# Totoro97/f2-nerf

Measured on AMD Instinct MI355X. Metric: training ray-samples/s (ngp_fox), higher is better.
Workload: dtype f16; 1 GPU; ngp_fox wanjinyou.yaml, 8192 rays/batch/GPU, 2^19 x16 table, the first 2188 iterations of training from the fresh-initialised table (fineness 8.7), synthetic random-pose rays, full train step (fwd+bwd+Adam+octree update); rays_per_batch=8192, parallelism=ray-dp1

## Files before the change

### f2-nerf_amd/capi.py

```python
import ctypes
import os

import torch

from . import build

_lib = None
ABI_VERSION = 13


class F2nError(RuntimeError):
    pass


def lib():
    global _lib
    if _lib is None:
        if not os.path.exists(build.LIB):
            raise F2nError("native library %s is missing: run `python -c 'import __graft_entry__ as g; g.build()'` "
                           "(there is no CPU fallback)" % build.LIB)
        _lib = ctypes.CDLL(build.LIB)
        _lib.f2n_build_info.restype = ctypes.c_char_p
        if _lib.f2n_abi_version() != ABI_VERSION:
            raise F2nError("%s reports ABI version %d, this binding is written for %d: rebuild (__graft_entry__.build())"
                           % (build.LIB, _lib.f2n_abi_version(), ABI_VERSION))
    return _lib


def _stream():
    return ctypes.c_void_p(torch.cuda.current_stream().cuda_stream)


_DT = {"f32": torch.float32, "i32": torch.int32, "i64": torch.int64, "u8": torch.uint8, "h16": torch.float16}


def _p(t, kind=None, allow_none=False):
    if t is None:
        if allow_none:
            return ctypes.c_void_p(0)
        raise F2nError("required tensor is None")
    if not t.is_cuda:
# ... 141 lines not shown
                                    _p(noise, "f32"), _p(oct_se, "i32"), _p(oct_idx, "i32"), _p(oct_nf, "f32"), _p(tree_nodes, "u8"),
                                    _p(transes, "u8"), _p(counts, "i32"), _p(s_pts, "f32", True), _p(s_dt, "f32"), _p(s_t, "f32"),
                                    _p(s_anchors, "i32"), _p(first_oct_dis, "f32"), _p(oct_trans, "i32", True)), "f2n_ray_march_strided")


def pack_samples(n_rays, pts_se, rays_o, rays_d, transes, s_pts, s_dt, s_t, s_anchors, pts, dirs, dt, t, anchors):
    _ck(lib().f2n_pack_samples(_stream(), _i(n_rays), _p(pts_se, "i32"), _p(rays_o, "f32", True), _p(rays_d, "f32"),
                               _p(transes, "u8", True), _p(s_pts, "f32", True), _p(s_dt, "f32"),
                               _p(s_t, "f32"), _p(s_anchors, "i32"), _p(pts, "f32"), _p(dirs, "f32"), _p(dt, "f32"), _p(t, "f32"),
                               _p(anchors, "i32")), "f2n_pack_samples")


def pack_samples_repair(n_rays, pts_se, rays_o, rays_d, transes, s_pts, s_dt, s_t, s_anchors, pts, dirs, dt, t, anchors, death_epoch,
                        spec_epoch):
    _ck(lib().f2n_pack_samples_repair(_stream(), _i(n_rays), _p(pts_se, "i32"), _p(rays_o, "f32", True), _p(rays_d, "f32"),
                                      _p(transes, "u8", True), _p(s_pts, "f32", True), _p(s_dt, "f32"), _p(s_t, "f32"),
                                      _p(s_anchors, "i32"), _p(pts, "f32"), _p(dirs, "f32"), _p(dt, "f32"), _p(t, "f32"),
                                      _p(anchors, "i32"), _p(death_epoch, "i32"), _i(spec_epoch)), "f2n_pack_samples_repair")


def edge_samples(n, edge_pool, transes, edge_idx, edge_coords, out_pts, out_idx):
    _ck(lib().f2n_edge_samples(_stream(), _i(n), _p(edge_pool, "u8"), _p(transes, "u8"), _p(edge_idx, "i32"),
                               _p(edge_coords, "f32"), _p(out_pts, "f32"), _p(out_idx, "i32")), "f2n_edge_samples")


def early_stop_votes(n_rays, pts_se, f0, f0_stride, dt, weights, alphas, mask, kept, anchors, anchor_stride, w_adder, a_adder, mark,
                     visit_cnt):
    _ck(lib().f2n_early_stop_votes(_stream(), _i(n_rays), _p(pts_se, "i32"), _p(f0, "f32"), _i(f0_stride), _p(dt, "f32"),
                                   _p(weights, "f32"), _p(alphas, "f32"), _p(mask, "i32"), _p(kept, "i32"), _i(w_adder.numel()),
                                   _p(anchors, "i32"), _i(anchor_stride), _p(w_adder, "i32"), _p(a_adder, "i32"), _p(mark, "i32"),
                                   _p(visit_cnt, "i32")), "f2n_early_stop_votes")


def oct_mark_visit(n_rays, pts_se, anchors, anchor_stride, weights, alphas, w_adder, a_adder, mark, visit_cnt):
    _ck(lib().f2n_oct_mark_visit(_stream(), _i(n_rays), _i(w_adder.numel()), _p(pts_se, "i32"), _p(anchors, "i32"), _i(anchor_stride),
                                 _p(weights, "f32"), _p(alphas, "f32"), _p(w_adder, "i32"), _p(a_adder, "i32"),
                                 _p(mark, "i32"), _p(visit_cnt, "i32")), "f2n_oct_mark_visit")


def oct_update_stats(n_nodes, w_adder, a_adder, mark, w_stats, a_stats, tree_nodes, child_blocks=None, reset_votes=False):
    _ck(lib().f2n_oct_update_stats(_stream(), _i(n_nodes), _p(w_adder, "i32"), _p(a_adder, "i32"), _p(mark, "i32"),
                                   _p(w_stats, "i32"), _p(a_stats, "i32"), _p(tree_nodes, "u8"),
                                   _p(child_blocks, "u8", True), _i(1 if reset_votes else 0)), "f2n_oct_update_stats")


def oct_update_stats_ex(n_nodes, w_adder, a_adder, mark, w_stats, a_stats, tree_nodes, child_blocks, reset_votes, died_at, epoch,
                        death_epoch):
    _ck(lib().f2n_oct_update_stats_ex(_stream(), _i(n_nodes), _p(w_adder, "i32"), _p(a_adder, "i32"), _p(mark, "i32"),
                                      _p(w_stats, "i32"), _p(a_stats, "i32"), _p(tree_nodes, "u8"), _p(child_blocks, "u8", True),
                                      _i(int(reset_votes)), _p(died_at, "i32", True), _i(epoch), _p(death_epoch, "i32", True),
                                      ctypes.c_void_p(0)), "f2n_oct_update_stats_ex")


def oct_intersect_repair(n_rays, max_hits, search_order, rays_o, rays_d, near, far, tree_nodes, oct_se, oct_idx, oct_nf, total,
                         oct_trans, child_blocks, died_at, spec_epoch, death_epoch, repair_flags, n_repaired=None):
    _ck(lib().f2n_oct_intersect_repair(_stream(), _i(n_rays), _i(max_hits), _p(search_order, "u8"), _p(rays_o, "f32"),
                                       _p(rays_d, "f32"), _f(near), _f(far), _p(tree_nodes, "u8"), _p(oct_se, "i32"),
                                       _p(oct_idx, "i32"), _p(oct_nf, "f32"), _p(total, "i32"), _p(oct_trans, "i32", True),
                                       _p(child_blocks, "u8", True), _p(died_at, "i32"), _i(spec_epoch), _p(death_epoch, "i32"),
                                       _p(repair_flags, "i32"), _p(n_repaired, "i32", True)), "f2n_oct_intersect_repair")


def ray_march_repair(n_rays, sample_l, scale_by_dis, rays_o, rays_d, noise, oct_se, oct_idx, oct_nf, tree_nodes, transes, counts,
                     s_pts, s_dt, s_t, s_anchors, first_oct_dis, oct_trans, repair_flags, death_epoch, spec_epoch):
    _ck(lib().f2n_ray_march_repair(_stream(), _i(n_rays), _f(sample_l), _i(int(scale_by_dis)), _p(rays_o, "f32"), _p(rays_d, "f32"),
                                   _p(noise, "f32"), _p(oct_se, "i32"), _p(oct_idx, "i32"), _p(oct_nf, "f32"), _p(tree_nodes, "u8"),
# ... 226 lines not shown


def draw_ray_batch(n_rays, u01, image_set, height, width, poses, intri, dist_params, images, cam_bounds, cam_indices, ij, rays_o,
                   rays_d, gt_colors, bounds):
    _ck(lib().f2n_draw_ray_batch(_stream(), _i(n_rays), _p(u01, "f32"), _p(image_set, "i32"), _i(int(image_set.numel())), _i(height),
                                 _i(width), _p(poses, "f32"), _p(intri, "f32"), _p(dist_params, "f32"), _p(images, "f32", True),
                                 _p(cam_bounds, "f32"), _p(cam_indices, "i32"), _p(ij, "i32"), _p(rays_o, "f32"), _p(rays_d, "f32"),
                                 _p(gt_colors, "f32", True), _p(bounds, "f32")), "f2n_draw_ray_batch")


def gather_pixels(n, height, width, images, cam_bounds, cam_idx, ij, gt_colors, bounds):
    _ck(lib().f2n_gather_pixels(_stream(), _i(n), _i(height), _i(width), _p(images, "f32", True), _p(cam_bounds, "f32", True),
                                _p(cam_idx, "i32"), _p(ij, "i32"), _p(gt_colors, "f32", True), _p(bounds, "f32", True)),
        "f2n_gather_pixels")


def early_stop(n_rays, pts_se, f0, f0_stride, dt, weights, alphas, mask, kept):
    _ck(lib().f2n_early_stop(_stream(), _i(n_rays), _p(pts_se, "i32"), _p(f0, "f32"), _i(f0_stride), _p(dt, "f32"),
                             _p(weights, "f32"), _p(alphas, "f32"), _p(mask, "i32"), _p(kept, "i32")), "f2n_early_stop")


def compact_samples(n_rays, old_se, new_se, mask, pts, dirs, dt, t, anchors, o_pts, o_dirs, o_dt, o_t, o_anchors):
    _ck(lib().f2n_compact_samples(_stream(), _i(n_rays), _p(old_se, "i32"), _p(new_se, "i32"), _p(mask, "i32"),
                                  _p(pts, "f32"), _p(dirs, "f32"), _p(dt, "f32"), _p(t, "f32"), _p(anchors, "i32"),
                                  _p(o_pts, "f32"), _p(o_dirs, "f32"), _p(o_dt, "f32"), _p(o_t, "f32"),
                                  _p(o_anchors, "i32")), "f2n_compact_samples")


def compact_samples_src(n_rays, old_se, new_se, mask, pts, dirs, dt, t, anchors, o_pts, o_dirs, o_dt, o_t, o_anchors, o_src,
                        o_vol=None, ray_val=None, o_ray_val=None):
    _ck(lib().f2n_compact_samples_src(_stream(), _i(n_rays), _p(old_se, "i32"), _p(new_se, "i32"), _p(mask, "i32"),
                                      _p(pts, "f32"), _p(dirs, "f32"), _p(dt, "f32"), _p(t, "f32"), _p(anchors, "i32"),
                                      _p(o_pts, "f32"), _p(o_dirs, "f32"), _p(o_dt, "f32"), _p(o_t, "f32"),
                                      _p(o_anchors, "i32"), _p(o_src, "i32"), _p(o_vol, "i32", True), _p(ray_val, "i32", True),
                                      _p(o_ray_val, "i32", True)), "f2n_compact_samples_src")


def oct_visible_cams(n_boxes, n_cams, boxes, c2w, bounds, fx, fy, cx, cy, res_h, res_w, pix_i, pix_j, visible):
    _ck(lib().f2n_oct_visible_cams(_stream(), _i(n_boxes), _i(n_cams), _p(boxes, "f32"), _p(c2w, "f32"), _p(bounds, "f32"), _f(fx),
                                   _f(fy), _f(cx), _f(cy), _i(res_h), _i(res_w), _p(pix_i, "f32"), _p(pix_j, "f32"),
                                   _p(visible, "u8")), "f2n_oct_visible_cams")


def march_noise(n, u, fineness, out):
    _ck(lib().f2n_march_noise(_stream(), _i(n), _p(u, "f32"), _f(fineness), _p(out, "f32")), "f2n_march_noise")


def composite_fwd(n_rays, pts_se, feat, dt, t, rgb, bg, colors, disparity, depth, weights, f0_stride=16, out_vars=None):
    _ck(lib().f2n_composite_fwd(_stream(), _i(n_rays), _p(pts_se, "i32"), _p(feat, "f32"), _i(f0_stride), _p(dt, "f32"),
                                _p(t, "f32"), _p(rgb, "f32"), _p(bg, "f32"), _p(colors, "f32"), _p(disparity, "f32"),
                                _p(depth, "f32"), _p(weights, "f32"), _p(out_vars, "f32", True)), "f2n_composite_fwd")


def composite_bwd(n_rays, pts_se, feat, dt, t, rgb, bg, dcolors, ddisp, ddepth, dweights, gs_progress, drgb, dfeat, f0_stride=16,
                  df0_stride=16, var_weights=None, dvars=None):
    _ck(lib().f2n_composite_bwd(_stream(), _i(n_rays), _p(pts_se, "i32"), _p(feat, "f32"), _i(f0_stride), _p(dt, "f32"),
                                _p(t, "f32"), _p(rgb, "f32"), _p(bg, "f32"), _p(dcolors, "f32", True), _p(ddisp, "f32", True),
                                _p(ddepth, "f32", True), _p(dweights, "f32", True), _f(gs_progress), _p(drgb, "f32"),
                                _p(dfeat, "f32"), _i(df0_stride), _p(var_weights, "f32", True), _p(dvars, "f32", True)),
        "f2n_composite_bwd")


def weight_var_fwd(n_rays, weights, pts_se, out):
    _ck(lib().f2n_weight_var_fwd(_stream(), _i(n_rays), _p(weights, "f32"), _p(pts_se, "i32"), _p(out, "f32")),
        "f2n_weight_var_fwd")


# ... 156 lines not shown


def reduce_deferred():
    _ck(lib().f2n_reduce_deferred(_stream()), "f2n_reduce_deferred")


def deferred_reset():
    _ck(lib().f2n_deferred_reset(), "f2n_deferred_reset")


def adam_step_h16grad(n, param, grad_h, grad_scale, exp_avg, exp_avg_sq, step, lr, beta1, beta2, eps, wd, param_h,
                      zero_grad, skip_flag=None):
    _ck(lib().f2n_adam_step_h16grad(_stream(), _i(n), _p(param, "f32"), _p(grad_h, "h16"), _f(grad_scale),
                                    _p(exp_avg, "f32"), _p(exp_avg_sq, "f32"), _i(step), _f(lr), _d(beta1), _d(beta2),
                                    _f(eps), _f(wd), _p(param_h, "h16"), _i(int(zero_grad)),
                                    _p(skip_flag, "i32", True)), "f2n_adam_step_h16grad")


def train_loss(n_rays, pred, gt, disparity, sampled_var, n_edge, feat_dim, edge_feats, var_w, disp_w, tv_w, out_losses,
               dcolors, ddisparity, dvar, dedge_feats):
    _ck(lib().f2n_train_loss(_stream(), _i(n_rays), _p(pred, "f32"), _p(gt, "f32"), _p(disparity, "f32", True),
                             _p(sampled_var, "f32", True), _i(n_edge), _i(feat_dim), _p(edge_feats, "f32", True), _f(var_w),
                             _f(disp_w), _f(tv_w), _p(out_losses, "f32"), _p(dcolors, "f32", True), _p(ddisparity, "f32", True),
                             _p(dvar, "f32", True), _p(dedge_feats, "f32", True)), "f2n_train_loss")


def composite_train(n_rays, se, f0, f0_stride, dt, t, rgb, bg, gt, var_w, disp_w, tv_w, gs_progress, n_edge, feat_dim, edge_feats,
                    dedge_feats, colors, weights, drgb, df0, df0_stride, out_losses, defer_reduce=False):
    _ck(lib().f2n_composite_train(_stream(), _i(n_rays), _p(se, "i32"), _p(f0, "f32"), _i(f0_stride), _p(dt, "f32"), _p(t, "f32"),
                                  _p(rgb, "f32"), _p(bg, "f32"), _p(gt, "f32"), _f(var_w), _f(disp_w), _f(tv_w), _f(gs_progress),
                                  _i(n_edge), _i(feat_dim), _p(edge_feats, "f32", True), _p(dedge_feats, "f32", True),
                                  _p(colors, "f32"), _p(weights, "f32"), _p(drgb, "f32"), _p(df0, "f32"), _i(df0_stride),
                                  _p(out_losses, "f32"), _i(1 if defer_reduce else 0)), "f2n_composite_train")


def nonfinite_flags(n_a, a, n_b, b, flags, mirror=None):
    _ck(lib().f2n_nonfinite_flags_ex(_stream(), _i(n_a), _p(a, "f32", True), _i(n_b), _p(b, "f32", True), _p(flags, "i32"),
                                     _mapped(mirror)), "f2n_nonfinite_flags_ex")


def _lo3(lo):
    return (_f * 3)(*(float(v) for v in lo))


def oct_locate_warp(n, pts_world, tree_nodes, transes, out_pts, out_anchors):
    _ck(lib().f2n_oct_locate_warp(_stream(), _i(n), _p(pts_world, "f32"), _p(tree_nodes, "u8"), _p(transes, "u8"), _p(out_pts, "f32"),
                                  _p(out_anchors, "i32")), "f2n_oct_locate_warp")


def oct_locate_warp_grid(lo, step, nx, ny, nz, first_z, n_z, tree_nodes, transes, out_pts, out_anchors):
    _ck(lib().f2n_oct_locate_warp_grid(_stream(), _lo3(lo), _f(step), _i(nx), _i(ny), _i(nz), _i(first_z), _i(n_z), _p(tree_nodes, "u8"),
                                       _p(transes, "u8"), _p(out_pts, "f32"), _p(out_anchors, "i32")), "f2n_oct_locate_warp_grid")


def located_compact(n, anchors, pts_warped, counts, start_end, total, out_pts, out_vol, out_src=None):
    _ck(lib().f2n_located_compact(_stream(), _i(n), _p(anchors, "i32"), _p(pts_warped, "f32"), _p(counts, "i32"), _p(start_end, "i32"),
                                  _p(total, "i32"), _p(out_pts, "f32"), _p(out_vol, "i32"), _p(out_src, "i32", True)),
        "f2n_located_compact")


def density_scatter(n, anchors, start_end, f0, density):
    _ck(lib().f2n_density_scatter(_stream(), _i(n), _p(anchors, "i32"), _p(start_end, "i32"), _p(f0, "f32"), _p(density, "f32")),
        "f2n_density_scatter")


def field_density_grad(n, n_volumes, table_h, prim_pool, local_idx, local_size, bias_pool, level_scale, pts_warped, volume_idx, vol_stride,
# ... 552 lines not shown
```

### f2-nerf_amd/csrc/host/PersSampler.cpp

```cpp
#include "PersSampler.h"

#include <hip/hip_runtime_api.h>

#include <algorithm>
#include <cstring>
#include <functional>

namespace f2n {

namespace {

Tensor BuildSearchOrder() {
  std::vector<int> search_order;
  for (int st = 0; st < 8; st++) {
    auto cmp = [st](int a, int b) {
      int bt = ((a ^ b) & -(a ^ b));
      return ((a & bt) ^ (st & bt)) != 0;
    };
    for (int i = 0; i < 8; i++) search_order.push_back(i);
    std::sort(search_order.begin() + st * 8, search_order.begin() + (st + 1) * 8, cmp);
  }
  return torch::from_blob(search_order.data(), {64}, CpuI32()).to(torch::kUInt8).to(torch::kCUDA).contiguous();
}

// ... 289 lines not shown
  F2N_CALL(f2n_edge_samples(CurStream(), n_pts, VoidP(pers_octree_->edge_pool_gpu_), VoidP(pers_octree_->pers_trans_gpu_),
                            I32P(edge_idx), F32P(edge_coord), F32P(out_pts), I32P(out_idx)));
  return {out_pts, out_idx};
}

Tensor& PersSampler::VoteBuffer() {
  auto& oct = *pers_octree_;
  const int n_nodes = oct.n_nodes_;
  Tensor& occ = oct.occ_;
  if (!occ.defined() || occ.size(1) != n_nodes || oct.tree_visit_cnt_.data_ptr() != (void*) (occ.data_ptr<int32_t>() + 3 * (int64_t) n_nodes)) {
    occ = torch::empty({4, n_nodes}, DevI32());
    occ.slice(0, 0, 2).fill_(-1);
    occ.select(0, 2).zero_();
    occ.select(0, 3).copy_(oct.tree_visit_cnt_);
    oct.tree_visit_cnt_ = occ.select(0, 3);
  }
  return occ;
}

void PersSampler::UpdateOctNodes(const SampleResultFlex& sample_result, const Tensor& sampled_weight,
                                 const Tensor& sampled_alpha) {
  const int n_nodes = pers_octree_->n_nodes_;
  const int n_rays = sample_result.pts_idx_bounds.size(0);
  CheckDev(sampled_weight, torch::kFloat32, "sampled_weight");
  CheckDev(sampled_alpha, torch::kFloat32, "sampled_alpha");
  Tensor& occ = VoteBuffer();
  F2N_TIMED_CALL("oct_mark_visit", f2n_oct_mark_visit(CurStream(), n_rays, n_nodes, I32P(sample_result.pts_idx_bounds), I32P(sample_result.anchors), 3,
                              F32P(sampled_weight), F32P(sampled_alpha), I32P(occ), I32P(occ) + n_nodes,
                              I32P(occ) + 2 * (int64_t) n_nodes, I32P(occ) + 3 * (int64_t) n_nodes));
  FinishOctUpdate();
}

void PersSampler::EarlyStopAndVote(const SampleResultFlex& sample_result, const float* f0, Tensor& weights, Tensor& alphas, Tensor& mask,
                                   Tensor& kept) {
  const int n_nodes = pers_octree_->n_nodes_;
  const int n_rays = sample_result.pts_idx_bounds.size(0);
  Tensor& occ = VoteBuffer();
  F2N_TIMED_CALL("early_stop", f2n_early_stop_votes(CurStream(), n_rays, I32P(sample_result.pts_idx_bounds), f0, 1, F32P(sample_result.dt),
                              F32P(weights), F32P(alphas), I32P(mask), I32P(kept), n_nodes, I32P(sample_result.anchors), 3, I32P(occ),
                              I32P(occ) + n_nodes, I32P(occ) + 2 * (int64_t) n_nodes, I32P(occ) + 3 * (int64_t) n_nodes));
}

void PersSampler::FinishOctUpdate(const ScanArgs* scan) {
  auto& oct = *pers_octree_;
  const int n_nodes = oct.n_nodes_;
  Tensor& occ = oct.occ_;
  void* st = CurStream();
  if (occupancy_sync_hook_) occupancy_sync_hook_(occ);
  Tensor adders = occ.slice(0, 0, 2), visit_mark = occ.select(0, 2);
  oct.epoch_++;
  if (scan != nullptr) {
    F2N_TIMED_CALL("oct_update_stats", f2n_oct_update_stats_scan(st, n_nodes, I32P(adders), I32P(adders) + n_nodes, I32P(visit_mark),
                                  I32P(oct.tree_weight_stats_), I32P(oct.tree_alpha_stats_), VoidP(oct.tree_nodes_gpu_),
                                  VoidP(oct.child_blocks_gpu_), 1, I32P(oct.died_at_), oct.epoch_, I32P(oct.death_epoch_),
                                  oct.death_epoch_host_dev_, scan->n, scan->counts, scan->start_end, scan->total, scan->mirror, scan->also,
                                  scan->n_also));
  } else {
    F2N_TIMED_CALL("oct_update_stats", f2n_oct_update_stats_ex(st, n_nodes, I32P(adders), I32P(adders) + n_nodes, I32P(visit_mark),
                                  I32P(oct.tree_weight_stats_), I32P(oct.tree_alpha_stats_), VoidP(oct.tree_nodes_gpu_),
                                  VoidP(oct.child_blocks_gpu_), 1, I32P(oct.died_at_), oct.epoch_, I32P(oct.death_epoch_),
                                  oct.death_epoch_host_dev_));
  }

  while (!sub_div_milestones_.empty() && sub_div_milestones_.back() <= global_data_pool_->iter_step_) {
    oct.ProcOctree(true, true, sub_div_milestones_.back() <= 0);
    oct.MarkInvisibleNodes();
    oct.ProcOctree(true, false, false);
    sub_div_milestones_.pop_back();
  }
  if (global_data_pool_->iter_step_ % compact_freq_ == 0) {
    oct.ProcOctree(true, false, false);
  }
}
// ... 113 lines not shown
```

### f2-nerf_amd/csrc/host/PersSampler.h

```cpp
#pragma once
#include <functional>

#include "KeyedDraws.h"
#include "MappedHost.h"
#include "PtsSampler.h"

namespace f2n {

#define INIT_NODE_STAT 1000
#define N_PROS 12

struct alignas(32) TransInfo {
  float w2xz[N_PROS][2][4];
  float weight[3][N_PROS];
  float center[3];
  float dis_summary;
};
struct alignas(32) TreeNode {
  float center[3];
  float side_len;
  int parent;
  int childs[8];
  bool is_leaf_node;
  int trans_idx;
// ... 52 lines not shown
  at::cuda::CUDAEvent counts_ready;
  bool speculative = false, completed = true;
  bool packed_once = false;
  int spec_epoch = 0;
  int64_t generation = 0;
  Tensor repair_flags;
  Tensor leaf_state, reached;
  bool tail = false;
};

class PersSampler : public PtsSampler {
 public:
  explicit PersSampler(GlobalDataPool* global_data_pool);
  SampleResultFlex GetSamples(const Tensor& rays_o, const Tensor& rays_d, const Tensor& bounds) override;
  void BeginSamples(const Tensor& rays_o, const Tensor& rays_d, float fineness, PendingSamples& p, bool speculative = false,
                    int64_t seq = -1);
  int64_t keyed_seq_ = -1;
  bool CompleteSpeculative(PendingSamples& p);
  void IssueScanAndPack(PendingSamples& p);
  void IssueScan(PendingSamples& p);
  bool tail_repair_ = true;
  int march_blocks_ = 512;
  int march_block_waves_ = 4;
  bool persistent_march_ = false;
  int LdsWalkMaxInterior() const { return f2n_oct_lds_max_interior(); }
  bool MaintenanceDue(int ahead = 0) const;
  bool MaintenanceDueAt(int iter) const;
  SampleResultFlex FinishSamples(PendingSamples& p);
  std::tuple<Tensor, Tensor> GetEdgeSamples(int n_pts) override;
  std::tuple<Tensor, Tensor> LocatePoints(const Tensor& world);
  void UpdateOctNodes(const SampleResultFlex& sample_result, const Tensor& sampled_weights,
                      const Tensor& sampled_alpha) override;
  void EarlyStopAndVote(const SampleResultFlex& sample_result, const float* f0, Tensor& weights, Tensor& alphas, Tensor& mask,
                        Tensor& kept);
  struct ScanArgs {
    int n = 0;
    const int32_t* counts = nullptr;
    int32_t *start_end = nullptr, *total = nullptr, *mirror = nullptr;
    const int32_t* also = nullptr;
    int n_also = 0;
  };
  void FinishOctUpdate(const ScanArgs* scan = nullptr);
  Tensor& VoteBuffer();
  MappedWords totals_words_;
  int next_totals_slot_ = 0;
  std::vector<Tensor> States() override;
  int LoadStates(const std::vector<Tensor>& states, int idx) override;

  void InstallOctree(const Tensor& tree_nodes_bytes, const Tensor& pers_trans_bytes, const Tensor& edge_pool_bytes);
  void SetEdgePool(const Tensor& edge_pool_bytes);
  void SetTrainCameras(const Tensor& w2c, const Tensor& intri, const Tensor& bounds);

  std::unique_ptr<PersOctree> pers_octree_;
  std::vector<int> sub_div_milestones_;
  int compact_freq_;
  int max_oct_intersect_per_ray_;
  float global_near_;
  float sample_l_;
  bool scale_by_dis_;
  std::function<void(Tensor)> occupancy_sync_hook_;
  Tensor forced_noise_, forced_edge_idx_, forced_edge_coords_;
  KeyedUniforms noise_draws_{0x9E3779B97F4A7C15ull};
  int extra_sample_rows_ = 0;
};

}
```

### f2-nerf_amd/csrc/host/Renderer.cpp

```cpp
#include "Renderer.h"

#include <hip/hip_runtime_api.h>

#include <cstdio>
#include <cstdlib>
#include <mutex>

namespace f2n {

using torch::autograd::AutogradContext;
using torch::autograd::variable_list;

namespace {

struct CompositeFunction : public torch::autograd::Function<CompositeFunction> {
  static variable_list forward(AutogradContext* ctx, Tensor feat, Tensor rgb, Tensor dt, Tensor t, Tensor bg, Tensor se,
                               double gs_progress) {
    ctx->set_materialize_grads(false);
    const int n_rays = se.size(0), m = feat.size(0);
    Tensor colors = torch::empty({n_rays, 3}, DevF32()), disparity = torch::empty({n_rays}, DevF32());
    Tensor depth = torch::empty({n_rays}, DevF32()), weights = torch::empty({m}, DevF32());
    F2N_TIMED_CALL("composite_fwd", f2n_composite_fwd(CurStream(), n_rays, I32P(se), F32P(feat), F2N_MLP_OUT_PAD, F32P(dt), F32P(t), F32P(rgb), F32P(bg),
                               F32P(colors), F32P(disparity), F32P(depth), F32P(weights), nullptr));
    ctx->save_for_backward({feat, rgb, dt, t, bg, se});
// ... 295 lines not shown
        vol_all = torch::empty({n_rows}, DevI32());
        edge_samples_to(F32P(pts_full), I32P(anchors_full), 3, F32P(pts_all), I32P(vol_all));
      }
      pack_done();
      if (digest_taps_ && train) {
        DigestTap(TAP_PTS_PRE, sample_result_.pts);
        DigestTap(TAP_DT_PRE, sample_result_.dt);
        DigestTap(TAP_ANCHORS_PRE, sample_result_.anchors.select(1, 0));
      }
      f0_full = field->QueryDensityPreAct(pts_full, anchors_full, true, keep_prepass_outputs_);
      f0p = F32P(f0_full) + front;
      if (digest_taps_ && train) DigestTap(TAP_EDGE, pts_full.narrow(0, 0, front));
      fr.edge_cache_row = 0;
      fr.sample_cache_row = front;
    } else {
      pack_done();
      if (digest_taps_ && train) {
        DigestTap(TAP_PTS_PRE, sample_result_.pts);
        DigestTap(TAP_DT_PRE, sample_result_.dt);
        DigestTap(TAP_ANCHORS_PRE, sample_result_.anchors.select(1, 0));
      }
      f0_full = field->QueryDensityPreAct(sample_result_.pts, sample_result_.anchors, true, keep_prepass_outputs_);
      f0p = F32P(f0_full);
    }
    if (digest_taps_ && train) {
      DigestTap(TAP_PTS, sample_result_.pts);
      DigestTap(TAP_DT, sample_result_.dt);
      DigestTap(TAP_ANCHORS, sample_result_.anchors.select(1, 0));
      DigestTap(TAP_F0, f0_full);
      DigestTap(TAP_BG, bg_color);
    }
    Tensor weights = torch::empty({n_all_pts}, DevF32()), alphas = torch::empty({n_all_pts}, DevF32());
    Tensor mask = torch::empty({n_all_pts}, DevI32()), kept = torch::empty({n_rays}, DevI32());
    if (train) ps->EarlyStopAndVote(sample_result_, f0p, weights, alphas, mask, kept);
    else F2N_TIMED_CALL("early_stop", f2n_early_stop(st, n_rays, I32P(sample_result_.pts_idx_bounds), f0p, 1, F32P(sample_result_.dt),
                            F32P(weights), F32P(alphas), I32P(mask), I32P(kept)));
    const bool octree_first = train && async_count;
    auto octree_update_issued = [&]() {
      octree_ready_ev_.record();
      const int nslot = next_batch_.valid ? FindPending(next_batch_.rays_o, next_batch_.rays_d) : -1;
      if (nslot >= 0 && pend_[nslot].s.speculative && !pend_[nslot].s.completed && PreSampleSpecComplete(nslot)) after_octree_update_ = nullptr;
      else if (nslot >= 0 && pend_[nslot].s.completed) after_octree_update_ = nullptr;
      if (after_octree_update_) {
        auto f = std::move(after_octree_update_);
        after_octree_update_ = nullptr;
        f();
      }
    };
    Tensor new_se = torch::empty({n_rays, 2}, DevI32()), total = torch::empty({1}, DevI32());
    n_kept_words_.Ensure(2);
    bool scan_issued = false;
    if (octree_first) {
      PersSampler::ScanArgs sa;
      sa.n = n_rays; sa.counts = I32P(kept); sa.start_end = I32P(new_se); sa.total = I32P(total);
      if (train && dp_world_ > 1 && dp_count_.defined()) {
        sa.mirror = n_kept_words_.Dev(0); sa.also = I32P(dp_count_); sa.n_also = 1;
        dp_sum_mirrored_ = true;
        dp_sum_rays_ = dp_count_rays_;
      } else {
        sa.mirror = n_kept_words_.Dev(1);
      }
      ps->FinishOctUpdate(&sa);
      scan_issued = true;
      octree_update_issued();
    }
    const bool dp_lagged = train && dp_world_ > 1 && octree_first;
    if (scan_issued) {
// ... 16 lines not shown
    if (train && !octree_first) ps->FinishOctUpdate();
    if (train && dp_world_ > 1 && !dp_lagged) {
      if (!dp_count_host_.defined()) dp_count_host_ = torch::empty({1}, torch::TensorOptions().dtype(torch::kInt32).pinned_memory(true));
      dp_count_host_.copy_(dp_count_, true);
      dp_count_ev_.record();
    }
    if (train && !octree_first) octree_update_issued();
    if (async_count) {
      n_kept = n_all_pts;
      if (train) {
        count_pending_ = true;
        pending_count_rays_ = n_rays;
        pending_count_seq_ = cur_seq_;
      }
      fr.dyn = true;
      fr.n_kept_dev = total;
    } else {
      kept_wait_ev_->synchronize();
      n_kept = n_kept_words_.Read(1);
      if (train && after_count_readback_) after_count_readback_();
      last_n_kept_pts_ = n_kept;
      if (train) total_kept_pts_ += n_kept;
    }
    const int64_t so = fr.dyn ? 2 * (int64_t) n_edge : 0;
    const int64_t eo = fr.dyn ? 0 : n_kept;
    if (!edges_cached) {
      pts_all = torch::empty({n_kept + 2 * n_edge, 3}, DevF32());
      vol_all = torch::empty({n_kept + 2 * n_edge}, DevI32());
    }
    es.pts = pts_all.slice(0, so, so + n_kept);
    es.dirs = torch::empty({n_kept, 3}, DevF32());
    es.dt = torch::empty({n_kept}, DevF32());
    es.t = torch::empty({n_kept}, DevF32());
    es.anchors = torch::empty({n_kept, 3}, DevI32());
    es.first_oct_dis = sample_result_.first_oct_dis;
    es.pts_idx_bounds = new_se;
    src_rows = torch::empty({std::max(n_kept, 1)}, DevI32());
    const bool want_emb = train && use_app_emb_ && emb_idx.defined();
    Tensor emb_contig;
    if (want_emb) {
      emb_contig = emb_idx.contiguous();
      CheckDev(emb_contig, torch::kInt32, "emb_idx");
      fr.sample_emb_idx = torch::empty({std::max(n_kept, 1)}, DevI32());
    }
    F2N_TIMED_CALL("compact_samples", f2n_compact_samples_src(st, n_rays, I32P(sample_result_.pts_idx_bounds), I32P(new_se), I32P(mask),
                                 F32P(sample_result_.pts), F32P(sample_result_.dirs), F32P(sample_result_.dt),
                                 F32P(sample_result_.t), I32P(sample_result_.anchors), F32P(pts_all) + 3 * so, F32P(es.dirs),
                                 F32P(es.dt), F32P(es.t), I32P(es.anchors), I32P(src_rows), I32P(vol_all) + so,
                                 want_emb ? I32P(emb_contig) : nullptr, want_emb ? I32P(fr.sample_emb_idx) : nullptr));
    if (train) {
      if (!fr.dyn) {
        gdp->meaningful_sampled_pts_per_ray_ = gdp->meaningful_sampled_pts_per_ray_ * 0.9f + KeptPerRayForEma(n_kept, n_rays) * 0.1f;
        RecordEma(cur_seq_);
        DigestKept(cur_seq_, n_kept);
      }
      if (!edges_cached && n_edge > 0) edge_samples_to(F32P(pts_all) + 3 * eo, I32P(vol_all) + eo, 1, nullptr, nullptr);
    }
  }

  fr.n_kept = n_kept;
  fr.n_edge = n_edge;
  fr.side_pool_buffers = pregen;
  fr.emb = train && use_app_emb_ && emb_idx.defined();
  if (!fr.emb) fr.sample_emb_idx = torch::empty({0}, DevI32());
  const bool streaming_train = train && fr.dyn;
  if (streaming_train && consumed_side_samples_) {
    fr.presamples_keepalive = std::move(sample_result_);
    fr.consumed_deferred = true;
    consumed_side_samples_ = false;
  }
  sample_result_ = SampleResultFlex();
  if (consumed_side_samples_) {
    side_shared_->consumed.record();
    consumed_side_samples_ = false;
    side_shared_->seq++;
  }
  if (!streaming_train) octree_ready_ev_.record();
  return fr;
}

RenderResult Renderer::Render(const Tensor& rays_o, const Tensor& rays_d, const Tensor& bounds, const Tensor& emb_idx) {
// ... 85 lines not shown
```

### f2-nerf_amd/csrc/host/Renderer.h

```cpp
#pragma once
#include "Hash3DAnchored.h"
#include "PersSampler.h"

namespace f2n {

class SHShader : public Shader {
 public:
  explicit SHShader(GlobalDataPool* global_data_pool);
  Tensor Query(const Tensor& feats, const Tensor& dirs) override;
  Tensor QueryFromField(const Tensor& field_feats, const Tensor& dirs, const Tensor& app_emb, const Tensor& sample_emb_idx,
                        Tensor* app_emb_grad);
  Tensor SHEncode(const Tensor& dirs);
  std::vector<Tensor> States() override;
  std::vector<ParamGroup> OptimParamGroups() override;
  int LoadStates(const std::vector<Tensor>& states, int idx) override;
  void Reset() override;

  std::unique_ptr<FusedMLP> mlp_;
  int d_hidden_, n_hiddens_, degree_;
  bool fused_ok_ = true;
};

struct RenderResult {
  Tensor colors;
// ... 208 lines not shown
    float value = 0.f;
  } ema_ring_[kEmaRing];
  void RecordEma(int64_t seq) {
    if (seq >= 0) ema_ring_[seq % kEmaRing] = {seq, global_data_pool_->meaningful_sampled_pts_per_ray_};
  }
  bool EmaAfter(int64_t seq, float* value) const {
    if (seq < 0 || ema_ring_[seq % kEmaRing].seq != seq) return false;
    *value = ema_ring_[seq % kEmaRing].value;
    return true;
  }
  int64_t pending_count_seq_ = -1;
  static constexpr int kDigestRing = 32768;
  struct StepDigest {
    int64_t seq = -1;
    int iter = 0, n_rays = 0, n_marched = 0, n_kept = -1;
  };
  std::vector<StepDigest> digest_;
  void DigestBegin(int n_rays, int n_marched) {
    if (cur_seq_ < 0) return;
    if (digest_.empty()) digest_.resize(kDigestRing);
    digest_[cur_seq_ % kDigestRing] = {cur_seq_, global_data_pool_->iter_step_, n_rays, n_marched, -1};
  }
  void DigestKept(int64_t seq, int n_kept) {
    if (seq >= 0 && !digest_.empty() && digest_[seq % kDigestRing].seq == seq) digest_[seq % kDigestRing].n_kept = n_kept;
  }
  enum { TAP_PTS, TAP_DT, TAP_ANCHORS, TAP_F0, TAP_SURVIVORS, TAP_BG, TAP_EDGE, TAP_COLORS, TAP_TABLE_GRAD, TAP_SMALL_GRADS, TAP_TABLE,
         TAP_FIELD_MLP, TAP_COLOR_MLP, TAP_APP_EMB, TAP_GRAD_BEFORE, TAP_PTS_ALL_AFTER, TAP_VOL_ALL_AFTER, TAP_FIELD_X, TAP_DFEAT,
         TAP_PTS_PRE, TAP_DT_PRE, TAP_ANCHORS_PRE, TAP_PTS_ALL_PRE, TAP_VOL_ALL_PRE, N_TAPS };
  bool digest_taps_ = false;
  Tensor digest_tap_sums_;
  void DigestTap(int tap, const Tensor& t);
  bool async_count_ = false;
  bool prepass_feat_reuse_ = true;
  bool keep_prepass_outputs_ = false;
  int64_t n_feat_reuse_steps_ = 0;
  bool count_pending_ = false;
  int pending_count_rays_ = 0;
  int64_t total_kept_pts_ = 0, total_all_pts_ = 0;
  TrainOutputs TrainForwardBackward(const Tensor& rays_o, const Tensor& rays_d, const Tensor& bounds, const Tensor& gt_colors,
                                    const Tensor& emb_idx, float var_w, float disp_w, float tv_w);

  Tensor QueryDensity(const Tensor& world);
  Tensor DensityGrid(const std::vector<float>& lo, const std::vector<float>& hi, int res);
  std::tuple<Tensor, Tensor> ExtractMesh(const std::vector<float>& lo, const std::vector<float>& hi, int res, float level);
  static GridSpec MakeGridSpec(const std::vector<float>& lo, const std::vector<float>& hi, int res);
  Tensor DensityOfLocated(const Tensor& warped, const Tensor& anchors);
  std::tuple<Tensor, Tensor> QueryRadiance(const Tensor& world, const Tensor& dirs);
  MeshAttrs ExtractMeshAttrs(const std::vector<float>& lo, const std::vector<float>& hi, int res, float level, int min_component_faces,
                             bool normals, bool colors, const std::string& normal_source = "grid", int simplify = 0,
                             const MeshRefineOptions& refine = MeshRefineOptions());
  LevelProjection ProjectToLevel(const Tensor& points, float level, int iters, float max_step, float max_move, float tol,
                                 const Tensor& origins = Tensor());
  std::tuple<Tensor, Tensor> QueryDensityGrad(const Tensor& world);
  Tensor FieldNormals(const Tensor& world);
  void DensityGradSlabs(const Tensor& world, const Tensor& density, const Tensor& grad, const Tensor& normals);
  void DensityGradChunk(const Tensor& world, const Tensor& density, const Tensor& grad, const Tensor& normals);
  GeometryResult RenderGeometry(const Tensor& rays_o, const Tensor& rays_d, const Tensor& bounds, float tau, bool keep_samples);
  int64_t density_slab_points_ = int64_t(1) << 22;

  int LoadStates(const std::vector<Tensor>& states, int idx) override;
  std::vector<Tensor> States() override;
  std::vector<ParamGroup> OptimParamGroups() override;
  void ZeroGrad();
  bool FusedPathOk() const;

  GlobalDataPool* global_data_pool_;
// ... 45 lines not shown
```

### f2-nerf_amd/csrc/host/RendererTrain.cpp

```cpp
#include "Renderer.h"

#include <hip/hip_runtime_api.h>

#include <cstdio>
#include <cstdlib>
#include <mutex>

namespace f2n {

using torch::autograd::AutogradContext;
using torch::autograd::variable_list;

TrainOutputs Renderer::TrainForwardBackward(const Tensor& rays_o, const Tensor& rays_d, const Tensor& bounds,
                                            const Tensor& gt_colors, const Tensor& emb_idx, float var_w, float disp_w, float tv_w) {
  auto* gdp = global_data_pool_;
  auto* field = static_cast<Hash3DAnchored*>(scene_field_.get());
  auto* shader = static_cast<SHShader*>(shader_.get());
  torch::NoGradGuard no_grad;
  const int n_rays = rays_o.size(0);
  Tensor gt = gt_colors.contiguous();
  CheckDev(gt, torch::kFloat32, "gt_colors");
  TORCH_CHECK(gt.numel() == (int64_t) n_rays * 3, "gt_colors must be [n_rays,3]");
  struct KeepOutputs {
    bool& flag;
// ... 40 lines not shown
    if (reuse) {
      x_cache = field->prepass_x_;
      feat_h_cache = field->prepass_feat_h_;
      n_feat_reuse_steps_++;
      const at::Half* fh = feat_h_cache.data_ptr<at::Half>();
      F2N_TIMED_CALL("field_shade_fwd", f2n_shade_fwd_feat(st, n_kept, n_dev, I32P(fr.src_rows),
                             static_cast<const void*>(fh + (int64_t) F2N_MLP_OUT_PAD * fr.sample_cache_row), F32P(es.dirs),
                             fr.emb ? F32P(app) : nullptr, fr.emb ? I32P(fr.sample_emb_idx) : nullptr, VoidP(shader->mlp_->params_h_),
                             F32P(f0c), VoidP(shade_x), F32P(rgb), edges_ride ? 2 * n_edge : 0,
                             edges_ride ? static_cast<const void*>(fh + (int64_t) F2N_MLP_OUT_PAD * fr.edge_cache_row) : nullptr,
                             edges_ride ? F32P(feat) : nullptr));
    } else {
      F2N_TIMED_CALL("field_shade_fwd", f2n_field_shade_fwd_extra(st, n_kept, n_dev, I32P(fr.src_rows),
                             static_cast<const void*>(cache + row * fr.sample_cache_row), VoidP(field->mlp_->params_h_), F32P(es.dirs),
                             fr.emb ? F32P(app) : nullptr, fr.emb ? I32P(fr.sample_emb_idx) : nullptr, VoidP(shader->mlp_->params_h_),
                             F32P(f0c), static_cast<void*>(field_x.data_ptr<at::Half>() + row * so), VoidP(shade_x), F32P(rgb),
                             edges_ride ? 2 * n_edge : 0, edges_ride ? static_cast<const void*>(cache + row * fr.edge_cache_row) : nullptr,
                             edges_ride ? F32P(feat) : nullptr, edges_ride ? VoidP(field_x) : nullptr));
    }
    field->DropPrepassCache();
  } else {
    field->ForwardRaw(fr.pts_all, fr.vol_all, 1, fr.src_rows, n_kept, feat, field_x, &f0c);
    field->DropPrepassCache();
    F2N_TIMED_CALL("shade_fwd", f2n_shade_fwd(st, n_kept, F32P(feat), F32P(es.dirs), fr.emb ? F32P(app) : nullptr,
                           fr.emb ? I32P(fr.sample_emb_idx) : nullptr, VoidP(shader->mlp_->params_h_), F32P(rgb), VoidP(shade_x)));
  }
  if (before_backward_) before_backward_();
  Tensor colors = torch::empty({n_rays, 3}, DevF32());
  Tensor weights = torch::empty({std::max(n_kept, 1)}, DevF32());
  Tensor bg = fr.bg_color.contiguous();
  Tensor dfeat = torch::empty({n, F2N_MLP_OUT_PAD}, DevF32());
  Tensor drgb = torch::empty({std::max(n_kept, 1), 3}, DevF32());
  if (fr.dyn) {
    F2N_TIMED_CALL("composite_train", f2n_composite_train(st, n_rays, I32P(es.pts_idx_bounds), F32P(f0c), 1, F32P(es.dt), F32P(es.t), F32P(rgb),
                                 F32P(bg), F32P(gt), var_w, disp_w, tv_w, gdp->gradient_scaling_progress_, n_edge, F2N_MLP_OUT_PAD,
                                 n_edge > 0 ? F32P(feat) + F2N_MLP_OUT_PAD * eo : nullptr, n_edge > 0 ? F32P(dfeat) + F2N_MLP_OUT_PAD * eo : nullptr,
                                 F32P(colors), F32P(weights), F32P(drgb), F32P(df0c), 1, F32P(out.losses), 1));
  } else {
    Tensor disparity = torch::empty({n_rays}, DevF32()), depth = torch::empty({n_rays}, DevF32());
    Tensor var = torch::empty({n_rays}, DevF32());
    F2N_TIMED_CALL("composite_fwd", f2n_composite_fwd(st, n_rays, I32P(es.pts_idx_bounds), F32P(f0c), 1, F32P(es.dt), F32P(es.t), F32P(rgb),
                               F32P(bg), F32P(colors), F32P(disparity), F32P(depth), F32P(weights), F32P(var)));

    Tensor dcolors = torch::empty({n_rays, 3}, DevF32()), ddisp = torch::empty({n_rays}, DevF32()), dvar = torch::empty({n_rays}, DevF32());
    F2N_TIMED_CALL("train_loss", f2n_train_loss(st, n_rays, F32P(colors), F32P(gt), F32P(disparity), F32P(var), n_edge, F2N_MLP_OUT_PAD,
                            F32P(feat) + F2N_MLP_OUT_PAD * eo, var_w, disp_w, tv_w, F32P(out.losses), F32P(dcolors),
                            F32P(ddisp), F32P(dvar), F32P(dfeat) + F2N_MLP_OUT_PAD * eo));

    F2N_TIMED_CALL("composite_bwd", f2n_composite_bwd(st, n_rays, I32P(es.pts_idx_bounds), F32P(f0c), 1, F32P(es.dt), F32P(es.t), F32P(rgb), F32P(bg),
                               F32P(dcolors), F32P(ddisp), nullptr, nullptr, gdp->gradient_scaling_progress_, F32P(drgb),
                               F32P(df0c), 1, F32P(weights), F32P(dvar)));
  }
  if (digest_taps_) DigestTap(TAP_GRAD_BEFORE, field->grad_h_);
  F2N_TIMED_CALL("shade_bwd", f2n_shade_bwd_dyn(st, n_kept, n_dev, F32P(drgb), fr.emb ? I32P(fr.sample_emb_idx) : nullptr,
                         VoidP(shader->mlp_->params_h_), VoidP(shade_x), shader->mlp_->loss_scale_, F32P(dfeat) + F2N_MLP_OUT_PAD * so,
                         F32P(shader->mlp_->grad_scaled_), fr.emb ? F32P(app_emb_grad_) : nullptr,
                         fr.emb ? (int) app_emb_grad_.size(0) : 0, F32P(df0c), fr.dyn ? 1 : 0));
  if (digest_taps_ && fr.dyn) {
    const int64_t rows = fr.pts_all.size(0);
    Tensor live = torch::arange(rows, DevI32()).lt(fr.n_kept_dev + (int) so).to(torch::kInt32);
    DigestTap(TAP_PTS_ALL_PRE, fr.pts_all.view(torch::kInt32).sum(1, false, torch::kInt64) * live);
    DigestTap(TAP_VOL_ALL_PRE, fr.vol_all.to(torch::kInt64) * live);
  }
  F2nStepTail tail;
  const bool fused_tail = fr.dyn && step_tail_builder_ && !digest_taps_ && step_tail_builder_(&tail);
  const int64_t xrow = (int64_t) N_LEVELS * N_CHANNELS;
  const void* x_edge = !reuse || n_edge == 0 ? nullptr
                       : edges_ride ? static_cast<const void*>(x_cache.data_ptr<at::Half>() + xrow * fr.edge_cache_row) : VoidP(field_x);
  const void* x_surv = reuse ? static_cast<const void*>(x_cache.data_ptr<at::Half>() + xrow * fr.sample_cache_row) : nullptr;
  if (fused_tail && reuse) {
// ... 59 lines not shown
```

### f2-nerf_amd/csrc/host/bindings.cpp

```cpp
#include <torch/extension.h>

#include "DataParallel.h"
#include "ExpRunner.h"

#include <hip/hip_runtime_api.h>

#include <algorithm>

using namespace f2n;

namespace {

Hash3DAnchored* FieldOf(ExpRunner& r) { return static_cast<Hash3DAnchored*>(r.renderer_->scene_field_.get()); }
SHShader* ShaderOf(ExpRunner& r) { return static_cast<SHShader*>(r.renderer_->shader_.get()); }
PersSampler* SamplerOf(ExpRunner& r) { return static_cast<PersSampler*>(r.renderer_->pts_sampler_.get()); }

struct InferenceMode {
  GlobalDataPool* gdp;
  RunningMode prev;
  InferenceMode(ExpRunner& r, bool on) : gdp(r.global_data_pool_.get()), prev(gdp->mode_) {
    if (on) gdp->mode_ = RunningMode::VALIDATE;
  }
  ~InferenceMode() { gdp->mode_ = prev; }
};
// ... 654 lines not shown
             }
             return out;
           })
      .def("step_digest",
           [](ExpRunner& r) {
             r.FinishPending();
             py::list out;
             auto& dg = r.renderer_->digest_;
             Tensor sums = r.digest_table_sums_.defined() ? r.digest_table_sums_.cpu() : Tensor();
             std::vector<Renderer::StepDigest> rows;
             for (auto& d : dg) if (d.seq >= 0) rows.push_back(d);
             std::sort(rows.begin(), rows.end(), [](const Renderer::StepDigest& a, const Renderer::StepDigest& b) { return a.seq < b.seq; });
             for (auto& d : rows) {
               py::list row;
               row.append(d.seq); row.append(d.iter); row.append(d.n_rays); row.append(d.n_marched); row.append(d.n_kept);
               if (sums.defined()) row.append(sums.data_ptr<int64_t>()[d.seq % Renderer::kDigestRing]);
               out.append(row);
             }
             return out;
           })
      .def_readwrite("iter_step", &ExpRunner::iter_step_)
      .def_readwrite("check_nan", &ExpRunner::check_nan_)
      .def_readwrite("async_counts", &ExpRunner::async_counts_)
      .def_property("speculative_sampling",
                    [](ExpRunner& r) { return r.renderer_->speculative_sampling_; },
                    [](ExpRunner& r, int mode) { r.renderer_->speculative_sampling_ = mode; })
      .def_property("tail_repair",
                    [](ExpRunner& r) { return static_cast<PersSampler*>(r.renderer_->pts_sampler_.get())->tail_repair_; },
                    [](ExpRunner& r, bool on) { static_cast<PersSampler*>(r.renderer_->pts_sampler_.get())->tail_repair_ = on; })
      .def_readwrite("fused_tail", &ExpRunner::fused_tail_)
      .def_property("prepass_feat_reuse",
                    [](ExpRunner& r) { return r.renderer_->prepass_feat_reuse_; },
                    [](ExpRunner& r, bool on) { r.renderer_->prepass_feat_reuse_ = on; })
      .def_property_readonly("prepass_reuse_steps", [](ExpRunner& r) { return r.renderer_->n_feat_reuse_steps_; })
      .def_readwrite("spec_start_without_event", &ExpRunner::spec_start_without_event_)
      .def_readwrite("draws_off_main", &ExpRunner::draws_off_main_)
      .def_readwrite("exact_flag_order", &ExpRunner::exact_flag_order_)
      .def_property("march_block_waves",
                    [](ExpRunner& r) { return static_cast<PersSampler*>(r.renderer_->pts_sampler_.get())->march_block_waves_; },
                    [](ExpRunner& r, int n) { static_cast<PersSampler*>(r.renderer_->pts_sampler_.get())->march_block_waves_ = std::min(16, std::max(1, n)); })
      .def_property("march_blocks",
                    [](ExpRunner& r) { return static_cast<PersSampler*>(r.renderer_->pts_sampler_.get())->march_blocks_; },
                    [](ExpRunner& r, int n) { static_cast<PersSampler*>(r.renderer_->pts_sampler_.get())->march_blocks_ = std::max(0, n); })
      .def_property("speculation_depth",
                    [](ExpRunner& r) { return r.renderer_->spec_depth_; },
                    [](ExpRunner& r, int d) { r.FinishPending(); r.renderer_->DropPendingSamples(); r.renderer_->spec_depth_ = std::max(1, std::min(3, d)); })
      .def("speculation_counters",
           [](ExpRunner& r) {
             r.FinishPending();
             py::dict d;
             d["speculative"] = r.renderer_->n_speculative_;
             d["fallback"] = r.renderer_->n_spec_fallback_;
             d["dropped"] = r.renderer_->n_spec_dropped_;
             auto& o = *SamplerOf(r)->pers_octree_;
             d["rays_repaired"] = o.n_repaired_.defined() ? o.n_repaired_.item<int>() : 0;
             d["stat_updates"] = o.epoch_;
             return d;
           })
      .def("counters",
           [](ExpRunner& r) {
             r.FinishPending();
             py::dict d;
             d["total_meaningful"] = r.renderer_->total_kept_pts_;
             d["total_marched"] = r.renderer_->total_all_pts_;
             return d;
           })
// ... 10 lines not shown
```

### f2-nerf_amd/csrc/render.hip

```cpp
#include "rows_dev.h"


__global__ __launch_bounds__(256) void early_stop_kernel(int n_rays, const int32_t* __restrict__ se, const float* __restrict__ f0,
                                                         int f0_stride, const float* __restrict__ dt, float* __restrict__ weights,
                                                         float* __restrict__ alphas, int32_t* __restrict__ mask,
                                                         int32_t* __restrict__ kept) {
  F2N_RAISE_PRIO();
  const int c = threadIdx.x & 15;
  const int ray = blockIdx.x * F2N_ROW_RAYS_PER_BLOCK + (threadIdx.x >> 4);
  if (ray >= n_rays) return;
  const int s = se[2 * ray], e = se[2 * ray + 1];
  float acc = 0.f;
  int cnt = 0;
  float n_f0 = 0.f, n_dt = 0.f;
  if (s < e) {
    const int i = min(s + c, e - 1);
    n_f0 = f0[(size_t) i * f0_stride];
    n_dt = dt[i];
  }
  for (int base = s; base < e; base += 16) {
    const int i = base + c;
    const bool in = i < e;
    const float c_f0 = n_f0, c_dt = n_dt;
    if (base + 16 < e) {
// ... 15 lines not shown
    }
    cnt += m;
  }
#pragma unroll
  for (int off = 8; off >= 1; off >>= 1) cnt += __shfl_xor(cnt, off, 16);
  if (c == 0) kept[ray] = cnt;
}

__global__ __launch_bounds__(256) void compact_kernel(int n_rays, const int32_t* __restrict__ old_se,
                                                      const int32_t* __restrict__ new_se, const int32_t* __restrict__ mask,
                                                      const float* __restrict__ pts, const float* __restrict__ dirs,
                                                      const float* __restrict__ dt, const float* __restrict__ t,
                                                      const int32_t* __restrict__ anchors, float* __restrict__ o_pts,
                                                      float* __restrict__ o_dirs, float* __restrict__ o_dt, float* __restrict__ o_t,
                                                      int32_t* __restrict__ o_anchors, int32_t* __restrict__ o_src,
                                                      int32_t* __restrict__ o_vol, const int32_t* __restrict__ ray_val,
                                                      int32_t* __restrict__ o_ray_val) {
  const int lane = threadIdx.x & 63;
  const int ray = blockIdx.x * (blockDim.x / 64) + (threadIdx.x >> 6);
  if (ray >= n_rays) return;
  const int s = old_se[2 * ray], e = old_se[2 * ray + 1];
  int dst = new_se[2 * ray];
  const int rv = o_ray_val != nullptr ? ray_val[ray] : 0;
  for (int base = s; base < e; base += 64) {
    const int i = base + lane;
    const bool keep = i < e && mask[i] != 0;
    const unsigned long long bal = __ballot(keep);
    if (keep) {
      const int k = dst + __popcll(bal & ((1ull << lane) - 1ull));
#pragma unroll
      for (int c = 0; c < 3; c++) {
        o_pts[3 * (size_t) k + c] = pts[3 * (size_t) i + c];
        o_dirs[3 * (size_t) k + c] = dirs[3 * (size_t) i + c];
        o_anchors[3 * (size_t) k + c] = anchors[3 * (size_t) i + c];
      }
      o_dt[k] = dt[i];
      o_t[k] = t[i];
      if (o_src != nullptr) o_src[k] = i;
      if (o_vol != nullptr) o_vol[k] = anchors[3 * (size_t) i];
      if (o_ray_val != nullptr) o_ray_val[k] = rv;
    }
    dst += __popcll(bal);
  }
}

__device__ __forceinline__ void f2n_wv_stats(const float* __restrict__ w, int n, int c, float& mean, float& wsum) {
  float m = 0.f, ws = 1e-6f;
  for (int base = 0; base < n; base += 16) {
    const int i = base + c;
    const float wi = i < n ? w[i] : 0.f;
    m = f2n_row_last(f2n_row_seq_scan(wi * ((float) i / 16.f), m, c));
    ws = f2n_row_last(f2n_row_seq_scan(wi, ws, c));
  }
  mean = m / ws;
  wsum = ws;
}

__global__ __launch_bounds__(256) void composite_fwd_kernel(int n_rays, const int32_t* __restrict__ se, const float* __restrict__ f0,
                                                            int f0_stride, const float* __restrict__ dt, const float* __restrict__ t,
                                                            const float* __restrict__ rgb, const float* __restrict__ bg,
                                                            float* __restrict__ colors, float* __restrict__ disparity,
                                                            float* __restrict__ depth, float* __restrict__ weights,
                                                            float* __restrict__ out_vars) {
  F2N_RAISE_PRIO();
  const int c = threadIdx.x & 15;
  const int ray = blockIdx.x * F2N_ROW_RAYS_PER_BLOCK + (threadIdx.x >> 4);
  if (ray >= n_rays) return;
// ... 178 lines not shown
    const float ems = expf(-sec);
    const float alpha = 1.f - ems;
    const float w = trans * alpha;
    float dw = (dC[0] * c0 + dC[1] * c1 + dC[2] * c2) + dDisp / tt + dDepW * tt;
    if (dweights != nullptr) dw += dwi;
    if (with_var && in) {
      const float r = (float) (i - s) / 16.f, b = r - wv_mean;
      dw += wv_dv * (b * b + wv_tmp * -r / wv_ws);
    }
    const float d_acc = in ? -dw * w : 0.f;
    const float suf_incl = f2n_row_seq_scan(d_acc, suffix, c);
    const float suf_i = f2n_row_exclusive(suf_incl, suffix, c);
    suffix = f2n_row_last(suf_incl);
    if (in) {
      const float d_sec = dw * trans * ems + suf_i + d_total;
      float d_sigma = d_sec * dti;
      float g0 = dC[0] * w, g1 = dC[1] * w, g2 = dC[2] * w;
      if (gs_progress < 1.f) {
        const float a = ((float) (i - s) + .5f) / (float) (e - s);
        const float sc = gs_progress + (1.f - gs_progress) * a * a;
        d_sigma *= sc;
        g0 *= sc; g1 *= sc; g2 *= sc;
      }
      drgb[3 * (size_t) i] = g0;
      drgb[3 * (size_t) i + 1] = g1;
      drgb[3 * (size_t) i + 2] = g2;
      df0[(size_t) i * df0_stride] = d_sigma * expf(fminf(fmaxf(x, -100.f), 5.f));
    }
  }
}


#define F2N_CT_TERMS 8
template <bool COLORS_IN>
__global__ __launch_bounds__(256) void composite_train_kernel(
    int n_rays, const int32_t* __restrict__ se, const float* __restrict__ f0, int f0_stride, const float* __restrict__ dt,
    const float* __restrict__ t, const float* __restrict__ rgb, const float* __restrict__ bg, const float* __restrict__ gt,
    float var_w, float disp_w, float tv_w, float gs_progress, int n_edge, int feat_dim, const float* __restrict__ edge,
    float* __restrict__ dedge, float* __restrict__ colors, float* __restrict__ weights, float* __restrict__ drgb,
    float* __restrict__ df0, int df0_stride, float* __restrict__ partials, float* __restrict__ out_losses, int ray_blocks,
    const float* __restrict__ colors_in) {
  F2N_RAISE_PRIO();
  __shared__ float s_terms[F2N_ROW_RAYS_PER_BLOCK][4];
  __shared__ float s_tv[256];
  if (blockIdx.x == 0 && threadIdx.x < F2N_CT_TERMS) out_losses[threadIdx.x] = 0.f;
  if ((int) blockIdx.x >= ray_blocks) {
    const int n_tv = n_edge * feat_dim;
    const float inv_tv = 1.f / (float) max(n_tv, 1);
    const int tvb = gridDim.x - ray_blocks;
    float acc = 0.f;
    for (int i = (blockIdx.x - ray_blocks) * 256 + threadIdx.x; i < n_tv; i += tvb * 256) {
      const int e = i / feat_dim, f = i - e * feat_dim;
      const size_t i0 = ((size_t) 2 * e) * feat_dim + f, i1 = i0 + feat_dim;
      const float d = edge[i0] - edge[i1];
      acc += d * d;
      if (dedge != nullptr) {
        const float g = tv_w * 2.f * d * inv_tv;
        dedge[i0] = g;
        dedge[i1] = -g;
      }
    }
    s_tv[threadIdx.x] = acc;
    __syncthreads();
    for (int off = 128; off >= 1; off >>= 1) {
      if ((int) threadIdx.x < off) s_tv[threadIdx.x] += s_tv[threadIdx.x + off];
      __syncthreads();
    }
    if (threadIdx.x < F2N_CT_TERMS) {
      const float tv = s_tv[0] * inv_tv;
      partials[(size_t) blockIdx.x * F2N_CT_TERMS + threadIdx.x] = threadIdx.x == 0 ? tv * tv_w : threadIdx.x == 4 ? tv : 0.f;
    }
    return;
  }
  const int c = threadIdx.x & 15, row = threadIdx.x >> 4;
  const int ray = blockIdx.x * F2N_ROW_RAYS_PER_BLOCK + row;
  const bool live = ray < n_rays;
  int s = 0, e = 0;
  if (live) {
    s = se[2 * ray];
    e = se[2 * ray + 1];
  }
  float acc = 0.f, col[3] = {0.f, 0.f, 0.f}, disp = 0.f, dep = 0.f, wv_m = 0.f, wv_ws = 1e-6f;
  {
    struct In {
      float f0, dt, t, c0, c1, c2;
    };
    auto fetch = [&](int i) {
      In r;
      r.f0 = f0[(size_t) i * f0_stride];
      r.dt = dt[i];
      r.t = t[i];
      if (!COLORS_IN) {
        r.c0 = rgb[3 * (size_t) i];
        r.c1 = rgb[3 * (size_t) i + 1];
        r.c2 = rgb[3 * (size_t) i + 2];
      } else {
        r.c0 = r.c1 = r.c2 = 0.f;
      }
      return r;
    };
    In nxt = {0.f, 0.f, 0.f, 0.f, 0.f, 0.f};
    if (s < e) nxt = fetch(min(s + c, e - 1));
    for (int base = s; base < e; base += 16) {
      const int i = base + c;
      const bool in = i < e;
      const In cur = nxt;
      if (base + 16 < e) nxt = fetch(min(i + 16, e - 1));
      float sec = 0.f, tt = 1.f, cr[3] = {0.f, 0.f, 0.f};
      if (in) {
        sec = expf(cur.f0 - F2N_DENSITY_SHIFT) * cur.dt;
        tt = cur.t + F2N_T_BIAS;
        cr[0] = cur.c0; cr[1] = cur.c1; cr[2] = cur.c2;
      }
      const float alpha = 1.f - expf(-sec);
      float excl;
      f2n_row_chain1x(sec, acc, excl);
      const float trans = expf(-excl);
      const float w = in ? trans * alpha : 0.f;
      if (in) weights[i] = w;
      const float x_disp = w / tt, x_dep = w * tt, x_m = w * ((float) (i - s) / 16.f);
      if (!COLORS_IN) {
        f2n_row_chain4(w * cr[0], w * cr[1], w * cr[2], x_disp, col[0], col[1], col[2], disp);
        f2n_row_chain3(x_dep, x_m, w, dep, wv_m, wv_ws);
      } else {
        f2n_row_chain4(x_disp, x_dep, x_m, w, disp, dep, wv_m, wv_ws);
      }
    }
    acc = f2n_row_last(acc);
#pragma unroll
    for (int k = 0; k < 3; k++) col[k] = f2n_row_last(col[k]);
    disp = f2n_row_last(disp);
    dep = f2n_row_last(dep);
    wv_m = f2n_row_last(wv_m);
    wv_ws = f2n_row_last(wv_ws);
  }
  if (COLORS_IN && live) {
#pragma unroll
    for (int k = 0; k < 3; k++) col[k] = colors_in[3 * ray + k];
  }
  const float total = acc;
  const float last_trans = expf(-total);
  float bgc[3] = {0.f, 0.f, 0.f}, gtc[3] = {0.f, 0.f, 0.f};
  if (live) {
#pragma unroll
    for (int k = 0; k < 3; k++) {
      bgc[k] = bg[3 * ray + k];
      gtc[k] = gt[3 * ray + k];
    }
  }
  float pred[3];
#pragma unroll
  for (int k = 0; k < 3; k++) pred[k] = col[k] + last_trans * bgc[k];
  if (live && c < 3) colors[3 * ray + c] = c == 0 ? pred[0] : c == 1 ? pred[1] : pred[2];
  float var = 0.f, wv_tmp = 0.f;
  const float wv_mean = wv_m / wv_ws;
  if (s < e) {
    float n_w = weights[min(s + c, e - 1)];
    for (int base = 0; base + s < e; base += 16) {
      const int i = base + c;
      const float c_w = n_w;
      if (base + 16 + s < e) n_w = weights[min(i + 16 + s, e - 1)];
      const float b = (float) i / 16.f - wv_mean;
      const float wi = i + s < e ? c_w : 0.f;
      f2n_row_chain2(wi * b * b, wi * 2.f * b, var, wv_tmp);
    }
    var = f2n_row_last(var);
    wv_tmp = f2n_row_last(wv_tmp);
  }
  const float inv_col = 1.f / (float) max(3 * n_rays, 1), inv_ray = 1.f / (float) max(n_rays, 1);
  float dC[3], t_col = 0.f, t_mse = 0.f;
#pragma unroll
  for (int k = 0; k < 3; k++) {
    const float d = pred[k] - gtc[k];
    const float r = sqrtf(d * d + 1e-4f);
    t_col += r;
    t_mse += d * d;
    dC[k] = d / r * inv_col;
  }
  const float r_var = sqrtf(var + 1e-2f);
  const float wv_dv = var_w * .5f / r_var * inv_ray;
  const float dDisp = disp_w * 2.f * disp * inv_ray;
  if (c == 0) {
    s_terms[row][0] = live ? t_col * inv_col : 0.f;
    s_terms[row][1] = live ? r_var * inv_ray : 0.f;
    s_terms[row][2] = live ? disp * disp * inv_ray : 0.f;
    s_terms[row][3] = live ? t_mse * inv_col : 0.f;
  }
  __syncthreads();
  if (threadIdx.x < F2N_CT_TERMS) {
    float sc = 0.f, sv = 0.f, sd = 0.f, sm = 0.f;
    for (int r = 0; r < F2N_ROW_RAYS_PER_BLOCK; r++) {
      sc += s_terms[r][0];
      sv += s_terms[r][1];
      sd += s_terms[r][2];
      sm += s_terms[r][3];
    }
    const int k = threadIdx.x;
    partials[(size_t) blockIdx.x * F2N_CT_TERMS + k] =
        k == 0 ? sc + sv * var_w + sd * disp_w : k == 1 ? sc : k == 2 ? sv : k == 3 ? sd : k == 5 ? sm : 0.f;
  }
  if (s >= e) return;
  const float dep_sum = dep;
  const float denom = 1.f - last_trans + 1e-4f;
  const float dDep = 0.f;
  const float d_last = (dC[0] * bgc[0] + dC[1] * bgc[1] + dC[2] * bgc[2]) + dDep * dep_sum / (denom * denom);
  const float d_total = -last_trans * d_last;
  const float dDepW = dDep / denom;
  struct RIn {
    float f0, dt, t, c0, c1, c2;
  };
  auto rfetch = [&](int i) {
    RIn r;
    r.f0 = f0[(size_t) i * f0_stride];
    r.dt = dt[i];
    r.t = t[i];
    r.c0 = rgb[3 * (size_t) i];
    r.c1 = rgb[3 * (size_t) i + 1];
    r.c2 = rgb[3 * (size_t) i + 2];
    return r;
  };
  float suffix = 0.f;
  RIn rn = rfetch(max(e - 1 - c, s));
  for (int hi = e; hi > s; hi -= 16) {
    const int i = hi - 1 - c;
    const bool in = i >= s;
    const RIn rc = rn;
    if (hi - 16 > s) rn = rfetch(max(i - 16, s));
    float x = 0.f, dti = 0.f, sigma = 0.f, tt = 1.f, c0 = 0.f, c1 = 0.f, c2 = 0.f;
    if (in) {
      x = rc.f0 - F2N_DENSITY_SHIFT;
      sigma = expf(x);
      dti = rc.dt;
      tt = rc.t + F2N_T_BIAS;
      c0 = rc.c0; c1 = rc.c1; c2 = rc.c2;
    }
    const float sec = in ? sigma * dti : 0.f;
    f2n_row_chain1(-sec, acc);
    const float acc_i = acc;
    const float trans = expf(-acc_i);
    const float ems = expf(-sec);
    const float alpha = 1.f - ems;
    const float w = trans * alpha;
    float dw = (dC[0] * c0 + dC[1] * c1 + dC[2] * c2) + dDisp / tt + dDepW * tt;
    if (in) {
      const float r = (float) (i - s) / 16.f, b = r - wv_mean;
      dw += wv_dv * (b * b + wv_tmp * -r / wv_ws);
    }
    const float d_acc = in ? -dw * w : 0.f;
    float suf_i;
    f2n_row_chain1x(d_acc, suffix, suf_i);
    if (in) {
      const float d_sec = dw * trans * ems + suf_i + d_total;
      float d_sigma = d_sec * dti;
      float g0 = dC[0] * w, g1 = dC[1] * w, g2 = dC[2] * w;
      if (gs_progress < 1.f) {
        const float a = ((float) (i - s) + .5f) / (float) (e - s);
        const float sc = gs_progress + (1.f - gs_progress) * a * a;
        d_sigma *= sc;
        g0 *= sc; g1 *= sc; g2 *= sc;
      }
      drgb[3 * (size_t) i] = g0;
      drgb[3 * (size_t) i + 1] = g1;
      drgb[3 * (size_t) i + 2] = g2;
      df0[(size_t) i * df0_stride] = d_sigma * expf(fminf(fmaxf(x, -100.f), 5.f));
    }
  }
}

__global__ __launch_bounds__(256) void weight_var_fwd_kernel(int n_rays, const float* __restrict__ weights,
                                                             const int32_t* __restrict__ se, float* __restrict__ out) {
  const int c = threadIdx.x & 15;
  const int ray = blockIdx.x * F2N_ROW_RAYS_PER_BLOCK + (threadIdx.x >> 4);
  if (ray >= n_rays) return;
  const int s = se[2 * ray], e = se[2 * ray + 1];
  if (s >= e) {
    if (c == 0) out[ray] = 0.f;
    return;
  }
  float mean, ws;
  f2n_wv_stats(weights + s, e - s, c, mean, ws);
  float var = 0.f;
  for (int base = 0; base + s < e; base += 16) {
    const int i = base + c;
    const float b = (float) i / 16.f - mean;
    const float wi = i + s < e ? weights[i + s] : 0.f;
    var = f2n_row_last(f2n_row_seq_scan(wi * b * b, var, c));
  }
  if (c == 0) out[ray] = var;
}

__global__ __launch_bounds__(256) void weight_var_bwd_kernel(int n_rays, const float* __restrict__ weights,
                                                             const int32_t* __restrict__ se, const float* __restrict__ dvars,
                                                             float* __restrict__ dw) {
  const int c = threadIdx.x & 15;
  const int ray = blockIdx.x * F2N_ROW_RAYS_PER_BLOCK + (threadIdx.x >> 4);
  if (ray >= n_rays) return;
  const int s = se[2 * ray], e = se[2 * ray + 1];
// ... 195 lines not shown
int f2n_compact_samples_src(void* stream, int n_rays, const int32_t* old_start_end, const int32_t* new_start_end,
                            const int32_t* mask, const float* pts, const float* dirs, const float* dt, const float* t,
                            const int32_t* anchors, float* o_pts, float* o_dirs, float* o_dt, float* o_t, int32_t* o_anchors,
                            int32_t* o_src, int32_t* o_vol, const int32_t* ray_val, int32_t* o_ray_val) {
  if (n_rays < 0 || o_src == nullptr || (o_ray_val != nullptr && ray_val == nullptr)) return F2N_ERR_INVALID_ARG;
  if (n_rays == 0) return F2N_OK;
  hipLaunchKernelGGL(compact_kernel, dim3(f2n_div_up(n_rays, 4)), dim3(256), 0, (hipStream_t) stream, n_rays, old_start_end,
                     new_start_end, mask, pts, dirs, dt, t, anchors, o_pts, o_dirs, o_dt, o_t, o_anchors, o_src, o_vol, ray_val,
                     o_ray_val);
  return f2n_launch_status();
}

int f2n_composite_fwd(void* stream, int n_rays, const int32_t* pts_start_end, const float* f0, int f0_stride, const float* dt,
                      const float* t, const float* rgb, const float* bg, float* colors, float* disparity, float* depth,
                      float* weights, float* out_vars) {
  if (f0_stride < 1) return F2N_ERR_INVALID_ARG;
  F2N_ROW_LAUNCH(composite_fwd_kernel, n_rays, pts_start_end, f0, f0_stride, dt, t, rgb, bg, colors, disparity, depth, weights,
                 out_vars);
}

int f2n_composite_bwd(void* stream, int n_rays, const int32_t* pts_start_end, const float* f0, int f0_stride, const float* dt,
                      const float* t, const float* rgb, const float* bg, const float* dcolors, const float* ddisparity,
                      const float* ddepth, const float* dweights, float grad_scaling_progress, float* drgb, float* df0,
                      int df0_stride, const float* var_weights, const float* dvars) {
  if (f0_stride < 1 || df0_stride < 1 || ((var_weights == nullptr) != (dvars == nullptr))) return F2N_ERR_INVALID_ARG;
  F2N_ROW_LAUNCH(composite_bwd_kernel, n_rays, pts_start_end, f0, f0_stride, dt, t, rgb, bg, dcolors, ddisparity, ddepth, dweights,
                 grad_scaling_progress, drgb, df0, df0_stride, var_weights, dvars);
}

static int f2n_composite_train_impl(void* stream, int n_rays, const int32_t* pts_start_end, const float* f0, int f0_stride, const float* dt,
                        const float* t, const float* rgb, const float* bg, const float* gt_colors, float var_w, float disp_w, float tv_w,
                        float grad_scaling_progress, int n_edge, int feat_dim, const float* edge_feats, float* dedge_feats,
                        float* colors, float* weights, float* drgb, float* df0, int df0_stride, float* out_losses, int defer_reduce,
                        const float* colors_in) {
  if (n_rays < 1 || f0_stride < 1 || df0_stride < 1 || n_edge < 0 || (n_edge > 0 && (edge_feats == nullptr || feat_dim < 1)) ||
      out_losses == nullptr)
    return F2N_ERR_INVALID_ARG;
  const int ray_blocks = (int) f2n_div_up(n_rays, F2N_ROW_RAYS_PER_BLOCK);
  const int tv_blocks = n_edge > 0 ? (int) min((long) 32, (long) f2n_div_up((long) n_edge * feat_dim, 256)) : 0;
  const int blocks = ray_blocks + tv_blocks;
  float* partials = (float*) f2n_ws_get(F2N_WS_LOSS, sizeof(float) * ((size_t) blocks * F2N_CT_TERMS + 64 * 8 + 16));
  if (partials == nullptr) return F2N_ERR_INVALID_ARG;
  partials += 64 * 8 + 16;
#if F2N_DEBUG_BUILD
  if (colors_in != nullptr)
    hipLaunchKernelGGL(composite_train_kernel<true>, dim3(blocks), dim3(256), 0, (hipStream_t) stream, n_rays, pts_start_end, f0, f0_stride, dt,
                       t, rgb, bg, gt_colors, var_w, disp_w, tv_w, grad_scaling_progress, n_edge, feat_dim, edge_feats, dedge_feats, colors,
                       weights, drgb, df0, df0_stride, partials, out_losses, ray_blocks, colors_in);
  else
#endif
  hipLaunchKernelGGL(composite_train_kernel<false>, dim3(blocks), dim3(256), 0, (hipStream_t) stream, n_rays, pts_start_end, f0, f0_stride, dt,
                     t, rgb, bg, gt_colors, var_w, disp_w, tv_w, grad_scaling_progress, n_edge, feat_dim, edge_feats, dedge_feats, colors,
                     weights, drgb, df0, df0_stride, partials, out_losses, ray_blocks, colors_in);
  const int rc = f2n_launch_status();
  if (rc != F2N_OK) return rc;
  if (defer_reduce) return f2n_defer_reduction(F2N_CT_TERMS, blocks, partials, out_losses);
  return f2n_reduce_partials(stream, F2N_CT_TERMS, blocks, partials, out_losses);
}

int f2n_composite_train(void* stream, int n_rays, const int32_t* pts_start_end, const float* f0, int f0_stride, const float* dt,
                        const float* t, const float* rgb, const float* bg, const float* gt_colors, float var_w, float disp_w, float tv_w,
                        float grad_scaling_progress, int n_edge, int feat_dim, const float* edge_feats, float* dedge_feats,
                        float* colors, float* weights, float* drgb, float* df0, int df0_stride, float* out_losses, int defer_reduce) {
  return f2n_composite_train_impl(stream, n_rays, pts_start_end, f0, f0_stride, dt, t, rgb, bg, gt_colors, var_w, disp_w, tv_w,
                                  grad_scaling_progress, n_edge, feat_dim, edge_feats, dedge_feats, colors, weights, drgb, df0, df0_stride,
                                  out_losses, defer_reduce, nullptr);
}

#if F2N_DEBUG_BUILD
int f2n_debug_composite_train_colors_in(void* stream, int n_rays, const int32_t* pts_start_end, const float* f0, int f0_stride,
                                        const float* dt, const float* t, const float* rgb, const float* bg, const float* gt_colors,
                                        float var_w, float disp_w, float tv_w, float grad_scaling_progress, float* colors, float* weights,
                                        float* drgb, float* df0, float* out_losses, const float* colors_in) {
  return f2n_composite_train_impl(stream, n_rays, pts_start_end, f0, f0_stride, dt, t, rgb, bg, gt_colors, var_w, disp_w, tv_w,
                                  grad_scaling_progress, 0, 16, nullptr, nullptr, colors, weights, drgb, df0, 1, out_losses, 0, colors_in);
}
#endif

int f2n_weight_var_fwd(void* stream, int n_rays, const float* weights, const int32_t* pts_start_end, float* out_vars) {
  F2N_ROW_LAUNCH(weight_var_fwd_kernel, n_rays, weights, pts_start_end, out_vars);
}

int f2n_weight_var_bwd(void* stream, int n_rays, const float* weights, const int32_t* pts_start_end, const float* dvars,
                       float* dweights) {
  F2N_ROW_LAUNCH(weight_var_bwd_kernel, n_rays, weights, pts_start_end, dvars, dweights);
}

int f2n_composite_geometry(void* stream, int n_rays, const int32_t* pts_start_end, const float* weights, const float* t, const float* rays_o,
                           const float* rays_d, const int32_t* anchors, const void* transes, const float* df0_dw, float tau,
                           float* out_opacity, float* out_normal, int32_t* out_surf_idx, float* out_surf_t, float* out_surf_point,
                           float* out_surf_normal, float* out_sample_grad, float* out_sample_normal) {
  if (!(tau > 0.f && tau <= 1.f)) return F2N_ERR_INVALID_ARG;
  if (n_rays > 0 && (pts_start_end == nullptr || weights == nullptr || t == nullptr || rays_o == nullptr || rays_d == nullptr ||
                     anchors == nullptr || transes == nullptr || df0_dw == nullptr || out_opacity == nullptr || out_normal == nullptr ||
                     out_surf_idx == nullptr || out_surf_t == nullptr || out_surf_point == nullptr || out_surf_normal == nullptr))
    return F2N_ERR_INVALID_ARG;
  F2N_ROW_LAUNCH(composite_geometry_kernel, n_rays, pts_start_end, weights, t, rays_o, rays_d, anchors, (const F2nTransInfo*) transes, df0_dw,
                 tau, out_opacity, out_normal, out_surf_idx, out_surf_t, out_surf_point, out_surf_normal, out_sample_grad, out_sample_normal);
}

int f2n_flex_sum_fwd(void* stream, int n_rays, int vec, const float* val, const int32_t* start_end, float* sum) {
  if (vec < 1) return F2N_ERR_INVALID_ARG;
  F2N_RAY_LAUNCH(flex_sum_fwd_kernel, n_rays, vec, val, start_end, sum);
}
int f2n_flex_sum_bwd(void* stream, int n_rays, int vec, const float* dsum, const int32_t* start_end, float* dval) {
  if (vec < 1) return F2N_ERR_INVALID_ARG;
  F2N_RAY_LAUNCH(flex_sum_bwd_kernel, n_rays, vec, dsum, start_end, dval);
}
// ... 9 lines not shown
```

### f2-nerf_amd/csrc/rows_dev.h

```cpp
#pragma once
#include "f2n_dev.h"

#define F2N_DENSITY_SHIFT 3.f
#define F2N_T_EPS 1e-4f
#define F2N_T_BIAS 1e-2f

#define F2N_ROW_RAYS_PER_BLOCK 16

__device__ __forceinline__ float f2n_row_shr1(float v) {
  return __int_as_float(__builtin_amdgcn_update_dpp(0, __float_as_int(v), 0x111, 0xF, 0xF, false));
}
#if defined(__HIP_DEVICE_COMPILE__)
#define F2N_DPP_STEP_(P, X) "v_add_f32_dpp " P ", " P ", " X " row_shr:1 row_mask:0xf bank_mask:0xf\n\t"
#define F2N_REP15_(S) S S S S S S S S S S S S S S S
__device__ __forceinline__ float f2n_row_seq_scan(float x, float carry, int c) {
  float p = carry + x;
  asm volatile("s_nop 4\n\t" F2N_REP15_(F2N_DPP_STEP_("%0", "%1") "s_nop 1\n\t") : "+v"(p) : "v"(x));
  return p;
}
#define F2N_DPP_HEAD_(P, X) "v_add_f32_dpp " P ", " P ", " X " row_ror:1 row_mask:0xf bank_mask:0xf\n\t"
__device__ __forceinline__ void f2n_row_chain1(float x, float& p) {
  asm volatile("s_nop 4\n\t" F2N_DPP_HEAD_("%0", "%1") "s_nop 1\n\t" F2N_REP15_(F2N_DPP_STEP_("%0", "%1") "s_nop 1\n\t") : "+v"(p) : "v"(x));
}
__device__ __forceinline__ void f2n_row_chain1x(float x, float& p, float& excl) {
// ... 27 lines not shown
  float p = carry + x;
#pragma unroll
  for (int k = 1; k < 16; k++) {
    const float t = f2n_row_shr1(p) + x;
    p = (c == 0) ? p : t;
  }
  return p;
}
__device__ __forceinline__ float f2n_row_last_(float v) { return __shfl(v, 15, 16); }
__device__ __forceinline__ void f2n_row_chain1(float x, float& p) { p = f2n_row_seq_scan(x, f2n_row_last_(p), (int) (threadIdx.x & 15)); }
__device__ __forceinline__ void f2n_row_chain1x(float x, float& p, float& excl) {
  const int c = threadIdx.x & 15;
  const float carry = f2n_row_last_(p);
  p = f2n_row_seq_scan(x, carry, c);
  const float prev = f2n_row_shr1(p);
  excl = c == 0 ? carry : prev;
}
__device__ __forceinline__ void f2n_row_chain2(float x0, float x1, float& p0, float& p1) {
  f2n_row_chain1(x0, p0);
  f2n_row_chain1(x1, p1);
}
__device__ __forceinline__ void f2n_row_chain3(float x0, float x1, float x2, float& p0, float& p1, float& p2) {
  f2n_row_chain1(x0, p0);
  f2n_row_chain1(x1, p1);
  f2n_row_chain1(x2, p2);
}
__device__ __forceinline__ void f2n_row_chain4(float x0, float x1, float x2, float x3, float& p0, float& p1, float& p2, float& p3) {
  f2n_row_chain1(x0, p0);
  f2n_row_chain1(x1, p1);
  f2n_row_chain1(x2, p2);
  f2n_row_chain1(x3, p3);
}
#endif
__device__ __forceinline__ float f2n_row_last(float v) { return __shfl(v, 15, 16); }
__device__ __forceinline__ float f2n_row_exclusive(float incl, float carry, int c) {
  const float prev = f2n_row_shr1(incl);
  return c == 0 ? carry : prev;
}
```

### f2-nerf_amd/csrc/sampler.hip

```cpp
#include "rows_dev.h"

#include <stdlib.h>


__device__ __forceinline__ void f2n_slab(const float* o, const float* d, const float* c, float side, float& near_,
                                         float& far_) {
  float lo[3], hi[3];
  float hf = side * .5f;
#pragma unroll
  for (int i = 0; i < 3; i++) {
    const bool par = d[i] < 1e-6f && d[i] > -1e-6f, pos = d[i] > 0;
    const float cm = c[i] - hf, cp = c[i] + hf;
    const float qm = (cm - o[i]) / d[i], qp = (cp - o[i]) / d[i];
    const bool inside = o[i] > cm && o[i] < cp;
    lo[i] = par ? (inside ? -1e6f : 1e6f) : (pos ? qm : qp);
    hi[i] = par ? (inside ? 1e6f : -1e6f) : (pos ? qp : qm);
  }
  near_ = fmaxf(near_, fmaxf(lo[0], fmaxf(lo[1], lo[2])));
  far_ = fminf(far_, fminf(hi[0], fminf(hi[1], hi[2])));
}

#define F2N_COOP_RAYS_PER_BLOCK 32
#define F2N_COOP_STACK 72
template <int MODE, bool LDSREC = false>
// ... 730 lines not shown
  float a[3], b[3];
  f2n_warp(transes + e->t_idx_a, w, a);
  f2n_warp(transes + e->t_idx_b, w, b);
#pragma unroll
  for (int c = 0; c < 3; c++) {
    out_pts[6 * i + c] = a[c];
    out_pts[6 * i + 3 + c] = b[c];
  }
  out_idx[(size_t) (2 * i) * idx_stride] = e->t_idx_a;
  out_idx[(size_t) (2 * i + 1) * idx_stride] = e->t_idx_b;
  if (out_pts2 != nullptr) {
#pragma unroll
    for (int c = 0; c < 3; c++) {
      out_pts2[6 * i + c] = a[c];
      out_pts2[6 * i + 3 + c] = b[c];
    }
    out_idx2[(size_t) (2 * i) * idx_stride2] = e->t_idx_a;
    out_idx2[(size_t) (2 * i + 1) * idx_stride2] = e->t_idx_b;
  }
}

#define F2N_VOTE_CAP 96
__device__ __forceinline__ void f2n_vote_global(int32_t* w_adder, int32_t* a_adder, int32_t* mark, int32_t* cnt, int node, int vw, int va,
                                                int visits) {
  const int cw = __hip_atomic_load(w_adder + node, __ATOMIC_RELAXED, __HIP_MEMORY_SCOPE_AGENT);
  const int ca = __hip_atomic_load(a_adder + node, __ATOMIC_RELAXED, __HIP_MEMORY_SCOPE_AGENT);
  const int cc = __hip_atomic_load(cnt + node, __ATOMIC_RELAXED, __HIP_MEMORY_SCOPE_AGENT);
  const int cm = __hip_atomic_load(mark + node, __ATOMIC_RELAXED, __HIP_MEMORY_SCOPE_AGENT);
  if (cw < vw) atomicMax(w_adder + node, vw);
  if (ca < va) atomicMax(a_adder + node, va);
  if (cc < visits) atomicMax(cnt + node, visits);
  if (cm != 1) mark[node] = 1;
}
__device__ __forceinline__ void f2n_votes_flush_row(const uint2* list, int n, int c, int32_t* w_adder, int32_t* a_adder, int32_t* mark, int32_t* cnt) {
  for (int k = c; k < n; k += 16) {
    const uint2 r = list[k];
    f2n_vote_global(w_adder, a_adder, mark, cnt, (int) r.x, (r.y & 1u) ? 512 : -1, (r.y & 2u) ? 32 : -1, (int) (r.y >> 2));
  }
}
__device__ __forceinline__ void f2n_vote(int32_t* w_adder, int32_t* a_adder, int32_t* mark, int32_t* cnt, int node,
                                         float w, float a, float w_thres, float a_thres, int visits) {
  atomicMax(w_adder + node, w > w_thres ? 512 : -1);
  atomicMax(a_adder + node, a > a_thres ? 32 : -1);
  atomicMax(cnt + node, visits);
  if (mark != nullptr) mark[node] = 1;
}

__device__ __forceinline__ void f2n_ray_votes(int s, int e, int c, float mw, float ma, const int32_t* __restrict__ anchors,
                                              int anchor_stride, const float* weights, const float* alphas, int32_t* w_adder,
                                              int32_t* a_adder, int32_t* mark, int32_t* cnt, uint2* vote_list = nullptr) {
  int n_queued = 0;
  const float w_thres = fminf((float) ((double) mw * 0.1), (float) 0.01);
  const float a_thres = fminf((float) ((double) ma * 0.1), (float) 0.02);
  float carry_w = 0.f, carry_a = 0.f;
  int carry_start = s, carry_node = -1;
  auto rot1 = [](int v) { return __builtin_amdgcn_update_dpp(0, v, 0x121, 0xF, 0xF, false); };
  struct Chunk {
    int node;
    float w, a;
  };
  auto fetch_chunk = [&](int b) {
    const int j = min(b + c, e - 1);
    Chunk q;
    q.node = anchors[(size_t) j * anchor_stride + 1];
    q.w = weights[j];
    q.a = alphas[j];
    return q;
  };
  Chunk q0 = fetch_chunk(s), q1 = fetch_chunk(s + 16), q2 = fetch_chunk(s + 32), q3 = fetch_chunk(s + 48);
  for (int base = s; base < e; base += 16) {
    const int i = base + c;
    const bool in = i < e;
    const int ic = in ? i : e - 1;
    const int node = q0.node;
    const float c_w = q0.w, c_a = q0.a;
    q0 = q1;
    q1 = q2;
    q2 = q3;
    q3 = fetch_chunk(base + 64);
    const int n_node = q0.node;
    const int prev = __builtin_amdgcn_update_dpp(base > s ? carry_node : -1, node, 0x111, 0xF, 0xF, false);
    const int nx0 = __builtin_amdgcn_update_dpp(0, n_node, 0x12F, 0xF, 0xF, false);
    const int nxt = __builtin_amdgcn_update_dpp(nx0, node, 0x101, 0xF, 0xF, false);
    const int next = ic + 1 < e ? nxt : -1;
    const bool head = node != prev;
    float cw = fmaxf(0.f, c_w), ca = fmaxf(0.f, c_a);
    int start = head ? ic : (int) 0x80000000;
    if (c == 0 && !head) {
      cw = fmaxf(cw, carry_w);
      ca = fmaxf(ca, carry_a);
      start = carry_start;
    }
    int f = head ? 1 : 0;
#define F2N_SEGMAX_STEP(K)                                                                     \
  {                                                                                            \
    const float tw = __int_as_float(__builtin_amdgcn_update_dpp(0, __float_as_int(cw), 0x110 + K, 0xF, 0xF, false)); \
    const float ta = __int_as_float(__builtin_amdgcn_update_dpp(0, __float_as_int(ca), 0x110 + K, 0xF, 0xF, false)); \
    const int ts = __builtin_amdgcn_update_dpp((int) 0x80000000, start, 0x110 + K, 0xF, 0xF, false);              \
    const int tf = __builtin_amdgcn_update_dpp(1, f, 0x110 + K, 0xF, 0xF, false);                                 \
    if (c >= K && f == 0) {                                                                    \
      cw = fmaxf(cw, tw);                                                                      \
      ca = fmaxf(ca, ta);                                                                      \
      start = max(start, ts);                                                                  \
    }                                                                                          \
    if (c >= K) f |= tf;                                                                       \
  }
    F2N_SEGMAX_STEP(1)
    F2N_SEGMAX_STEP(2)
    F2N_SEGMAX_STEP(4)
    F2N_SEGMAX_STEP(8)
#undef F2N_SEGMAX_STEP
    const bool votes = in && node != next;
    if (vote_list == nullptr) {
      if (votes) f2n_vote(w_adder, a_adder, mark, cnt, node, cw, ca, w_thres, a_thres, ic - start + 1);
    } else {
      const unsigned row_bits = (unsigned) ((__ballot(votes) >> (threadIdx.x & 48)) & 0xFFFFull);
      const int n_new = __popc(row_bits);
      if (n_queued + n_new > F2N_VOTE_CAP) {
        f2n_votes_flush_row(vote_list, n_queued, c, w_adder, a_adder, mark, cnt);
        n_queued = 0;
      }
      if (votes)
        vote_list[n_queued + __popc(row_bits & ((1u << c) - 1u))] =
            make_uint2((unsigned) node, (cw > w_thres ? 1u : 0u) | (ca > a_thres ? 2u : 0u) | ((unsigned) (ic - start + 1) << 2));
      n_queued += n_new;
    }
    carry_w = __int_as_float(rot1(__float_as_int(cw)));
    carry_a = __int_as_float(rot1(__float_as_int(ca)));
    carry_start = rot1(start);
    carry_node = rot1(node);
  }
  if (vote_list != nullptr) f2n_votes_flush_row(vote_list, n_queued, c, w_adder, a_adder, mark, cnt);
}

__device__ __forceinline__ void f2n_votes_lds_init(int32_t* s_votes, int n_nodes) {
  for (int i = threadIdx.x; i < n_nodes; i += blockDim.x) {
    s_votes[i] = -2;
    s_votes[n_nodes + i] = -2;
    s_votes[2 * n_nodes + i] = 0;
  }
  __syncthreads();
}
__device__ __forceinline__ void f2n_votes_lds_flush(const int32_t* s_votes, int n_nodes, int32_t* g_w_adder, int32_t* g_a_adder,
                                                    int32_t* g_mark, int32_t* g_cnt) {
  __syncthreads();
  for (int i = threadIdx.x; i < n_nodes; i += blockDim.x) {
    const int visits = s_votes[2 * n_nodes + i];
    if (visits > 0) {
      atomicMax(g_w_adder + i, s_votes[i]);
      atomicMax(g_a_adder + i, s_votes[n_nodes + i]);
      atomicMax(g_cnt + i, visits);
      g_mark[i] = 1;
    }
  }
}

template <bool USE_LDS>
__global__ void mark_visit_kernel(int n_rays, int n_nodes, const int32_t* __restrict__ pts_start_end,
                                  const int32_t* __restrict__ anchors, int anchor_stride, const float* __restrict__ weights,
                                  const float* __restrict__ alphas, int32_t* g_w_adder, int32_t* g_a_adder, int32_t* g_mark,
                                  int32_t* g_cnt) {
  extern __shared__ int32_t s_votes[];
  __shared__ uint2 s_vote_list[USE_LDS ? 1 : 16 * F2N_VOTE_CAP];
  int32_t* w_adder = USE_LDS ? s_votes : g_w_adder;
  int32_t* a_adder = USE_LDS ? s_votes + n_nodes : g_a_adder;
  int32_t* cnt = USE_LDS ? s_votes + 2 * n_nodes : g_cnt;
  int32_t* mark = USE_LDS ? nullptr : g_mark;
  if (USE_LDS) f2n_votes_lds_init(s_votes, n_nodes);
  const int c = threadIdx.x & 15;
  const int ray = blockIdx.x * (blockDim.x >> 4) + (threadIdx.x >> 4);
  int s = 0, e = 0;
  if (ray < n_rays) {
    s = pts_start_end[2 * ray];
    e = pts_start_end[2 * ray + 1];
  }
  if (s < e) {
    float mw = 0.f, ma = 0.f;
    for (int i = s + c; i < e; i += 16) {
      mw = fmaxf(mw, weights[i]);
      ma = fmaxf(ma, alphas[i]);
    }
#pragma unroll
    for (int off = 8; off >= 1; off >>= 1) {
      mw = fmaxf(mw, __shfl_xor(mw, off, 16));
      ma = fmaxf(ma, __shfl_xor(ma, off, 16));
    }
    f2n_ray_votes(s, e, c, mw, ma, anchors, anchor_stride, weights, alphas, w_adder, a_adder, mark, cnt,
                  USE_LDS ? nullptr : s_vote_list + (threadIdx.x >> 4) * F2N_VOTE_CAP);
  }
  if (USE_LDS) f2n_votes_lds_flush(s_votes, n_nodes, g_w_adder, g_a_adder, g_mark, g_cnt);
}

template <bool USE_LDS>
__global__ void early_stop_votes_kernel(int n_rays, int n_nodes, const int32_t* __restrict__ se, const float* __restrict__ f0,
                                        int f0_stride, const float* __restrict__ dt, float* weights, float* alphas,
                                        int32_t* __restrict__ mask, int32_t* __restrict__ kept,
                                        const int32_t* __restrict__ anchors, int anchor_stride, int32_t* g_w_adder,
                                        int32_t* g_a_adder, int32_t* g_mark, int32_t* g_cnt) {
  extern __shared__ int32_t s_votes[];
  __shared__ uint2 s_vote_list[USE_LDS ? 1 : 16 * F2N_VOTE_CAP];
  int32_t* w_adder = USE_LDS ? s_votes : g_w_adder;
  int32_t* a_adder = USE_LDS ? s_votes + n_nodes : g_a_adder;
  int32_t* cnt_v = USE_LDS ? s_votes + 2 * n_nodes : g_cnt;
  int32_t* mark = USE_LDS ? nullptr : g_mark;
  if (USE_LDS) f2n_votes_lds_init(s_votes, n_nodes);
  const int c = threadIdx.x & 15;
  const int ray = blockIdx.x * (blockDim.x >> 4) + (threadIdx.x >> 4);
  int s = 0, e = 0;
  if (ray < n_rays) {
    s = se[2 * ray];
    e = se[2 * ray + 1];
  }
  float acc = 0.f, mw = 0.f, ma = 0.f;
  int cnt = 0;
  float n_f0 = 0.f, n_dt = 0.f;
  if (s < e) {
    const int i = min(s + c, e - 1);
    n_f0 = f0[(size_t) i * f0_stride];
    n_dt = dt[i];
  }
  for (int base = s; base < e; base += 16) {
    const int i = base + c;
    const bool in = i < e;
    const float c_f0 = n_f0, c_dt = n_dt;
    if (base + 16 < e) {
      const int j = min(i + 16, e - 1);
      n_f0 = f0[(size_t) j * f0_stride];
      n_dt = dt[j];
    }
    float sec = 0.f;
    if (in) sec = expf(c_f0 - F2N_DENSITY_SHIFT) * c_dt;
    const float alpha = 1.f - expf(-sec);
    float excl;
    f2n_row_chain1x(sec, acc, excl);
    const float trans = expf(-excl);
    const int m = (in && trans > F2N_T_EPS) ? 1 : 0;
    if (in) {
      const float w = trans * alpha;
      weights[i] = w;
      alphas[i] = alpha;
      mask[i] = m;
      mw = fmaxf(mw, w);
      ma = fmaxf(ma, alpha);
    }
    cnt += m;
  }
#pragma unroll
  for (int off = 8; off >= 1; off >>= 1) {
    cnt += __shfl_xor(cnt, off, 16);
    mw = fmaxf(mw, __shfl_xor(mw, off, 16));
    ma = fmaxf(ma, __shfl_xor(ma, off, 16));
  }
  if (ray < n_rays && c == 0) kept[ray] = cnt;
  if (s < e)
    f2n_ray_votes(s, e, c, mw, ma, anchors, anchor_stride, weights, alphas, w_adder, a_adder, mark, cnt_v,
                  USE_LDS ? nullptr : s_vote_list + (threadIdx.x >> 4) * F2N_VOTE_CAP);
  if (USE_LDS) f2n_votes_lds_flush(s_votes, n_nodes, g_w_adder, g_a_adder, g_mark, g_cnt);
}

struct F2nStatsArgs {
  int n_nodes;
  int32_t *w_adder, *a_adder, *mark, *w_stats, *a_stats;
  F2nTreeNode* nodes;
  F2nChildInfo* child_blocks;
  int reset_votes;
  int32_t* died_at;
  int epoch;
  int32_t *death_epoch, *death_epoch_host;
};

__device__ __forceinline__ void f2n_update_stats_node(int i, const F2nStatsArgs& a) {
  int32_t* __restrict__ w_adder = a.w_adder;
  int32_t* __restrict__ a_adder = a.a_adder;
  int32_t* __restrict__ mark = a.mark;
  int32_t* __restrict__ w_stats = a.w_stats;
  int32_t* __restrict__ a_stats = a.a_stats;
  F2nTreeNode* __restrict__ nodes = a.nodes;
  F2nChildInfo* __restrict__ child_blocks = a.child_blocks;
  int32_t* __restrict__ died_at = a.died_at;
  int32_t* __restrict__ death_epoch = a.death_epoch;
  int32_t* __restrict__ death_epoch_host = a.death_epoch_host;
  const int reset_votes = a.reset_votes, epoch = a.epoch, n_nodes = a.n_nodes;
  if (i >= n_nodes) return;
  const int m = mark[i];
  int st[2];
  const int add[2] = {w_adder[i], a_adder[i]};
  if (reset_votes) {
    w_adder[i] = -1;
    a_adder[i] = -1;
// ... 444 lines not shown
  return f2n_edge_samples_ex(stream, n_pts, edge_pool, 0, transes, edge_idx, edge_coords, nullptr, out_pts, out_idx, 1, nullptr,
                             nullptr, 1);
}

int f2n_edge_samples_ex(void* stream, int n_pts, const void* edge_pool, int n_edges, const void* transes, const int32_t* edge_idx,
                        const float* edge_coords, const float* u01, float* out_pts, int32_t* out_idx, int idx_stride,
                        float* out_pts2, int32_t* out_idx2, int idx_stride2) {
  if (n_pts < 0 || idx_stride < 1 || idx_stride2 < 1 || (u01 != nullptr && n_edges < 1) || (out_pts2 != nullptr) != (out_idx2 != nullptr))
    return F2N_ERR_INVALID_ARG;
  if (n_pts == 0) return F2N_OK;
  if (u01 == nullptr && (edge_idx == nullptr || edge_coords == nullptr)) return F2N_ERR_INVALID_ARG;
  hipLaunchKernelGGL(edge_samples_kernel, dim3(f2n_div_up(n_pts, 64)), dim3(64), 0, (hipStream_t) stream, n_pts,
                     (const F2nEdgePool*) edge_pool, n_edges, (const F2nTransInfo*) transes, edge_idx, edge_coords, u01, out_pts,
                     out_idx, idx_stride, out_pts2, out_idx2, idx_stride2);
  return f2n_launch_status();
}

int f2n_oct_mark_visit(void* stream, int n_rays, int n_nodes, const int32_t* pts_start_end, const int32_t* anchors,
                       int anchor_stride, const float* weights, const float* alphas, int32_t* w_adder, int32_t* a_adder,
                       int32_t* mark, int32_t* visit_cnt) {
  if (n_rays < 0 || n_nodes < 1 || anchor_stride < 2) return F2N_ERR_INVALID_ARG;
  if (n_rays == 0) return F2N_OK;
  const size_t lds = sizeof(int32_t) * 3 * (size_t) n_nodes;
  if (lds <= 60 * 1024) {
    hipLaunchKernelGGL(mark_visit_kernel<true>, dim3(f2n_div_up(n_rays, 64)), dim3(1024), lds, (hipStream_t) stream, n_rays,
                       n_nodes, pts_start_end, anchors, anchor_stride, weights, alphas, w_adder, a_adder, mark, visit_cnt);
  } else {
    hipLaunchKernelGGL(mark_visit_kernel<false>, dim3(f2n_div_up(n_rays, 16)), dim3(256), 0, (hipStream_t) stream, n_rays,
                       n_nodes, pts_start_end, anchors, anchor_stride, weights, alphas, w_adder, a_adder, mark, visit_cnt);
  }
  return f2n_launch_status();
}

int f2n_early_stop_votes(void* stream, int n_rays, const int32_t* pts_start_end, const float* f0, int f0_stride, const float* dt,
                         float* weights, float* alphas, int32_t* mask, int32_t* kept, int n_nodes, const int32_t* anchors,
                         int anchor_stride, int32_t* w_adder, int32_t* a_adder, int32_t* mark, int32_t* visit_cnt) {
  if (n_rays < 0 || n_nodes < 1 || anchor_stride < 2 || f0_stride < 1) return F2N_ERR_INVALID_ARG;
  if (n_rays == 0) return F2N_OK;
  const size_t lds = sizeof(int32_t) * 3 * (size_t) n_nodes;
  if (lds <= 60 * 1024) {
    hipLaunchKernelGGL(early_stop_votes_kernel<true>, dim3(f2n_div_up(n_rays, 64)), dim3(1024), lds, (hipStream_t) stream, n_rays,
                       n_nodes, pts_start_end, f0, f0_stride, dt, weights, alphas, mask, kept, anchors, anchor_stride, w_adder,
                       a_adder, mark, visit_cnt);
  } else {
    hipLaunchKernelGGL(early_stop_votes_kernel<false>, dim3(f2n_div_up(n_rays, 16)), dim3(256), 0, (hipStream_t) stream, n_rays,
                       n_nodes, pts_start_end, f0, f0_stride, dt, weights, alphas, mask, kept, anchors, anchor_stride, w_adder,
                       a_adder, mark, visit_cnt);
  }
  return f2n_launch_status();
}

int f2n_oct_update_stats(void* stream, int n_nodes, int32_t* w_adder, int32_t* a_adder, int32_t* mark, int32_t* w_stats,
                         int32_t* a_stats, void* tree_nodes, void* child_blocks, int reset_votes) {
  return f2n_oct_update_stats_ex(stream, n_nodes, w_adder, a_adder, mark, w_stats, a_stats, tree_nodes, child_blocks, reset_votes,
                                 nullptr, 0, nullptr, nullptr);
}

int f2n_oct_update_stats_ex(void* stream, int n_nodes, int32_t* w_adder, int32_t* a_adder, int32_t* mark, int32_t* w_stats,
                            int32_t* a_stats, void* tree_nodes, void* child_blocks, int reset_votes, int32_t* died_at, int epoch,
                            int32_t* death_epoch, int32_t* death_epoch_host) {
  if (n_nodes < 0 || (died_at != nullptr) != (death_epoch != nullptr)) return F2N_ERR_INVALID_ARG;
  if (n_nodes == 0) return F2N_OK;
  const F2nStatsArgs a = {n_nodes, w_adder, a_adder, mark, w_stats, a_stats, (F2nTreeNode*) tree_nodes, (F2nChildInfo*) child_blocks, reset_votes,
                          died_at, epoch, death_epoch, death_epoch_host};
  hipLaunchKernelGGL(update_stats_kernel, dim3(f2n_div_up(n_nodes, 256)), dim3(256), 0, (hipStream_t) stream, a);
  return f2n_launch_status();
}

int f2n_oct_update_stats_scan(void* stream, int n_nodes, int32_t* w_adder, int32_t* a_adder, int32_t* mark, int32_t* w_stats,
                              int32_t* a_stats, void* tree_nodes, void* child_blocks, int reset_votes, int32_t* died_at, int epoch,
                              int32_t* death_epoch, int32_t* death_epoch_host, int n, const int32_t* counts, int32_t* start_end,
                              int32_t* total, int32_t* mirror, const int32_t* also, int n_also) {
  if (n_nodes < 0 || (died_at != nullptr) != (death_epoch != nullptr) || n < 0 || n_also < 0 || n_also > 4 ||
      (n_also > 0 && (also == nullptr || mirror == nullptr)))
    return F2N_ERR_INVALID_ARG;
  const F2nStatsArgs a = {n_nodes, w_adder, a_adder, mark, w_stats, a_stats, (F2nTreeNode*) tree_nodes, (F2nChildInfo*) child_blocks, reset_votes,
                          died_at, epoch, death_epoch, death_epoch_host};
  hipLaunchKernelGGL(stats_and_scan_kernel, dim3(1 + f2n_div_up(n_nodes, F2N_SCAN_THREADS)), dim3(F2N_SCAN_THREADS), 0, (hipStream_t) stream, a,
                     n, counts, start_end, total, mirror, also, n_also);
  return f2n_launch_status();
}

// ... 19 lines not shown
```

### include/f2n_abi.h

```cpp
#ifndef F2N_ABI_H
#define F2N_ABI_H

#include <stdint.h>

#ifdef __cplusplus
extern "C" {
#endif

#define F2N_OK 0
#define F2N_ERR_INVALID_ARG (-1)
#define F2N_ERR_UNSUPPORTED (-2)

#define F2N_N_LEVELS 16
#define F2N_N_CHANNELS 2
#define F2N_MAX_SAMPLE_PER_RAY 1024
#define F2N_MLP_OUT_PAD 16

int f2n_abi_version(void);
int f2n_numerics_mode(void);
const char* f2n_build_info(void);
typedef void (*f2n_bucket_fn)(void* user, int bucket, int n_buckets);
int f2n_set_scatter_buckets(int n_buckets, f2n_bucket_fn fn, void* user);
int f2n_set_scatter_buckets_for(int n_buckets, f2n_bucket_fn fn, void* user, const void* grad_table_h16);
int f2n_debug_counters(int32_t* out8_host , int reset);
// ... 207 lines not shown
                          int32_t* size);
int f2n_oct_subdivide(void* stream, int n_nodes, const void* nodes, const int32_t* visit_cnt, int brute_force, const int32_t* size,
                      const int32_t* w_stats, const int32_t* a_stats, int32_t* new_idx, void* dst_nodes, int32_t* dst_w, int32_t* dst_a);

int f2n_field_fwd_cached_dyn(void* stream, int n_max, const int32_t* n_dev, int n_cache, const int32_t* src_rows,
                             const void* x_cache_h, const void* mlp_params_h, float* out_feat_f32, float* out_f0, void* save_x_h);
int f2n_field_bwd_dyn(void* stream, int n_max, const int32_t* n_dev, int n_off, int n_volumes, const int32_t* prim_pool,
                      const int32_t* local_idx, const int32_t* local_size, const float* bias_pool, const float* level_scale,
                      const float* pts_warped, const int32_t* volume_idx, int vol_stride, const void* mlp_params_h,
                      const void* saved_x_h, const float* dfeat, float loss_scale, float* dparams_f32_scaled, void* grad_table_h,
                      int level_entries, int defer_reduce);
int f2n_shade_fwd_dyn(void* stream, int n_max, const int32_t* n_dev, const float* feat, const float* dirs, const float* app_emb,
                      const int32_t* sample_emb_idx, const void* mlp_params_h, float* rgb, void* save_x_h);
int f2n_field_shade_fwd_dyn(void* stream, int n_max, const int32_t* n_dev, const int32_t* src_rows, const void* x_cache_h,
                            const void* field_params_h, const float* dirs, const float* app_emb, const int32_t* sample_emb_idx,
                            const void* color_params_h, float* out_f0, void* save_field_x_h, void* save_shade_x_h, float* rgb);
int f2n_field_shade_fwd_extra(void* stream, int n_max, const int32_t* n_dev, const int32_t* src_rows, const void* x_cache_h,
                              const void* field_params_h, const float* dirs, const float* app_emb, const int32_t* sample_emb_idx,
                              const void* color_params_h, float* out_f0, void* save_field_x_h, void* save_shade_x_h, float* rgb,
                              int n_extra, const void* x_extra_h, float* feat_extra, void* save_x_extra_h);
int f2n_shade_bwd_dyn(void* stream, int n_max, const int32_t* n_dev, const float* drgb, const int32_t* sample_emb_idx,
                      const void* mlp_params_h, const void* saved_x_h, float loss_scale, float* dfeat, float* dparams_f32_scaled,
                      float* dapp_emb, int n_emb, const float* df0, int defer_reduce);
int f2n_reduce_deferred(void* stream);
int f2n_deferred_reset(void);


int f2n_early_stop(void* stream, int n_rays, const int32_t* pts_start_end, const float* f0, int f0_stride,
                   const float* dt, float* weights , float* alphas , int32_t* mask ,
                   int32_t* kept );
int f2n_early_stop_votes(void* stream, int n_rays, const int32_t* pts_start_end, const float* f0, int f0_stride, const float* dt,
                         float* weights, float* alphas, int32_t* mask, int32_t* kept, int n_nodes, const int32_t* anchors,
                         int anchor_stride, int32_t* w_adder, int32_t* a_adder, int32_t* mark, int32_t* visit_cnt);

int f2n_compact_samples(void* stream, int n_rays, const int32_t* old_start_end, const int32_t* new_start_end,
                        const int32_t* mask, const float* pts, const float* dirs, const float* dt, const float* t,
                        const int32_t* anchors, float* o_pts, float* o_dirs, float* o_dt, float* o_t,
                        int32_t* o_anchors);
int f2n_compact_samples_src(void* stream, int n_rays, const int32_t* old_start_end, const int32_t* new_start_end,
                            const int32_t* mask, const float* pts, const float* dirs, const float* dt, const float* t,
                            const int32_t* anchors, float* o_pts, float* o_dirs, float* o_dt, float* o_t,
                            int32_t* o_anchors, int32_t* o_src ,
                            int32_t* o_vol ,
                            const int32_t* ray_val ,
                            int32_t* o_ray_val );

int f2n_composite_fwd(void* stream, int n_rays, const int32_t* pts_start_end, const float* f0, int f0_stride,
                      const float* dt, const float* t, const float* rgb , const float* bg ,
                      float* colors , float* disparity , float* depth , float* weights ,
                      float* out_vars );

int f2n_composite_bwd(void* stream, int n_rays, const int32_t* pts_start_end, const float* f0, int f0_stride,
                      const float* dt, const float* t, const float* rgb, const float* bg, const float* dcolors,
                      const float* ddisparity, const float* ddepth, const float* dweights,
                      float grad_scaling_progress, float* drgb, float* df0, int df0_stride,
                      const float* var_weights , const float* dvars );

int f2n_weight_var_fwd(void* stream, int n_rays, const float* weights, const int32_t* pts_start_end, float* out_vars);
int f2n_weight_var_bwd(void* stream, int n_rays, const float* weights, const int32_t* pts_start_end,
                       const float* dvars, float* dweights);

int f2n_flex_sum_fwd(void* stream, int n_rays, int vec, const float* val, const int32_t* start_end, float* sum);
int f2n_flex_sum_bwd(void* stream, int n_rays, int vec, const float* dsum, const int32_t* start_end, float* dval);
int f2n_flex_acc_fwd(void* stream, int n_rays, int include_this, const float* val, const int32_t* start_end, float* sum);
int f2n_flex_acc_bwd(void* stream, int n_rays, int include_this, const float* dsum, const int32_t* start_end, float* dval);

int f2n_img2world_rays(void* stream, int n_rays, const float* poses, const float* intri, const float* dist_params,
                       const int32_t* cam_indices , const int32_t* ij , float* rays_o ,
                       float* rays_d );
int f2n_gather_pixels(void* stream, int n_rays, int height, int width, const float* images, const float* cam_bounds,
                      const int32_t* cam_indices, const int32_t* ij, float* gt_colors , float* bounds );
int f2n_draw_ray_batch(void* stream, int n_rays, const float* u01, const int32_t* image_set, int n_set, int height, int width,
                       const float* poses, const float* intri, const float* dist_params, const float* images ,
                       const float* cam_bounds, int32_t* cam_indices, int32_t* ij, float* rays_o, float* rays_d,
                       float* gt_colors , float* bounds);
// ... 63 lines not shown
                           const int32_t* local_size, const float* bias_pool, const float* level_scale, const float* pts_warped,
                           const int32_t* volume_idx, int vol_stride, const void* mlp_params_h, float* out_feat_f32 ,
                           float* out_f0 , void* save_x_h , void* out_feat_h );
int f2n_field_mlp_planes_ex(void* stream, int n, const void* planes_h, const void* mlp_params_h, float* out_feat_f32,
                            float* out_f0, void* save_x_h, void* out_feat_h);
int f2n_shade_fwd_feat(void* stream, int n_max, const int32_t* n_dev, const int32_t* src_rows, const void* feat_cache_h,
                       const float* dirs, const float* app_emb, const int32_t* sample_emb_idx, const void* color_params_h,
                       float* out_f0, void* save_shade_x_h, float* rgb, int n_extra, const void* feat_extra_h, float* feat_extra);
int f2n_field_bwd_dyn_rows(void* stream, int n_max, const int32_t* n_dev, int n_off, int n_volumes, const int32_t* prim_pool,
                           const int32_t* local_idx, const int32_t* local_size, const float* bias_pool, const float* level_scale,
                           const float* pts_warped, const int32_t* volume_idx, int vol_stride, const void* mlp_params_h,
                           const void* x_edge_h, const void* x_cache_h, const int32_t* src_rows, const float* dfeat, float loss_scale,
                           float* dparams_f32_scaled, void* grad_table_h, int level_entries, int defer_reduce);
int f2n_field_bwd_step_tail_rows(void* stream, void* tail_stream , int n_max, const int32_t* n_dev, int n_off, int n_volumes,
                                 const int32_t* prim_pool, const int32_t* local_idx, const int32_t* local_size, const float* bias_pool,
                                 const float* level_scale, const float* pts_warped, const int32_t* volume_idx, int vol_stride,
                                 const void* mlp_params_h, const void* x_edge_h, const void* x_cache_h, const int32_t* src_rows,
                                 const float* dfeat, float loss_scale, float* dparams_f32_scaled, void* grad_table_h, int level_entries,
                                 const F2nStepTail* tail, int* table_stepped_by_owners );
int f2n_adam_step_h16grad(void* stream, int n, float* param, void* grad_h, float grad_scale, float* exp_avg,
                          float* exp_avg_sq, int step, float lr, double beta1, double beta2, float eps,
                          float weight_decay, void* param_h, int zero_grad, const int32_t* skip_flag );

int f2n_train_loss(void* stream, int n_rays, const float* pred_colors , const float* gt_colors ,
                   const float* disparity , const float* sampled_var , int n_edge, int feat_dim,
                   const float* edge_feats , float var_w, float disp_w, float tv_w,
                   float* out_losses , float* dcolors, float* ddisparity, float* dvar, float* dedge_feats);

int f2n_composite_train(void* stream, int n_rays, const int32_t* pts_start_end, const float* f0, int f0_stride, const float* dt,
                        const float* t, const float* rgb, const float* bg, const float* gt_colors, float var_w, float disp_w, float tv_w,
                        float grad_scaling_progress, int n_edge, int feat_dim, const float* edge_feats ,
                        float* dedge_feats , float* colors, float* weights, float* drgb, float* df0, int df0_stride,
                        float* out_losses , int defer_reduce);

int f2n_nonfinite_flags(void* stream, int n_a, const float* a, int n_b, const float* b, int32_t* flags );
int f2n_nonfinite_flags_ex(void* stream, int n_a, const float* a, int n_b, const float* b, int32_t* flags ,
                           int32_t* mirror );

int f2n_oct_locate_warp(void* stream, int n, const float* pts_world , const void* tree_nodes, const void* transes,
                        float* out_pts_warped , int32_t* out_anchors );
int f2n_oct_locate_warp_grid(void* stream, const float* lo , float step, int nx, int ny, int nz, int first_z, int n_z,
                             const void* tree_nodes, const void* transes, float* out_pts_warped ,
                             int32_t* out_anchors );
int f2n_located_compact(void* stream, int n, const int32_t* anchors , const float* pts_warped , int32_t* counts ,
                        int32_t* start_end , int32_t* total , float* out_pts , int32_t* out_vol ,
                        int32_t* out_src );
int f2n_density_scatter(void* stream, int n, const int32_t* anchors , const int32_t* start_end , const float* f0,
                        float* density );
int f2n_mesh_count(void* stream, int nx, int ny, int nz, const float* grid, float level, uint8_t* edge_mask ,
                   int32_t* vert_counts , int32_t* vert_start_end , int32_t* face_counts ,
                   int32_t* face_start_end , int32_t* totals );
int f2n_mesh_emit(void* stream, int nx, int ny, int nz, const float* grid, float level, const float* lo , float step,
                  const uint8_t* edge_mask, const int32_t* vert_start_end, const int32_t* face_start_end, float* verts, int32_t* faces);
int f2n_radiance_scatter(void* stream, int n, const int32_t* anchors , const int32_t* start_end , const float* f0,
                         const float* rgb_rows, float* density , float* rgb );
int f2n_grid_normals(void* stream, int n, const float* pts , const float* grid, int nx, int ny, int nz,
                     const float* lo , float step, float* out );
int f2n_mesh_components(void* stream, int n_verts, int n_faces, const int32_t* faces , int32_t* labels ,
                        int32_t* changed , int* rounds );
int f2n_mesh_filter_count(void* stream, int n_verts, int n_faces, const int32_t* faces , const int32_t* labels ,
                          int min_faces, int32_t* comp_faces , int32_t* vert_keep , int32_t* vert_start_end ,
                          int32_t* face_keep , int32_t* face_start_end , int32_t* totals );
int f2n_mesh_filter_emit(void* stream, int n_verts, int n_faces, const float* verts , const int32_t* faces ,
                         const int32_t* vert_keep, const int32_t* vert_start_end, const int32_t* face_keep, const int32_t* face_start_end,
                         float* out_verts, int32_t* vert_src, int32_t* out_faces);
int f2n_field_density_grad(void* stream, int n, int n_volumes, const void* table_h, const int32_t* prim_pool, const int32_t* local_idx,
// ... 103 lines not shown
```

Baseline: 667.1 million ray-samples/s.

## Add optional wave-wide ray walks for long rays and skip unused anchor compaction

Restructures the early-stop/vote and composite-train kernels into templated per-ray walk helpers that can process long rays with a full 64-lane wave instead of a 16-lane row, selected by a wave_walk setting. The aim is to reduce load imbalance from long rays. It also stops allocating and writing compacted anchors in dynamic training, where they are unused, which saves some memory traffic. The default wave_walk is 0, so the wave path stays off unless the setting is changed. The refactored helpers still add some code-path overhead.

```diff
diff --git a/f2-nerf_amd/capi.py b/f2-nerf_amd/capi.py
--- a/f2-nerf_amd/capi.py
+++ b/f2-nerf_amd/capi.py
@@ -7,6 +7,8 @@
 
 _lib = None
 ABI_VERSION = 13
+RAY_WALK_WAVE_DEFAULT = 0
+RAY_WALK_WAVE_FITTED = 16
 
 
 class F2nError(RuntimeError):
@@ -214,6 +216,14 @@
                                    _p(visit_cnt, "i32")), "f2n_early_stop_votes")
 
 
+def early_stop_votes_ex(n_rays, pts_se, f0, f0_stride, dt, weights, alphas, mask, kept, anchors, anchor_stride, w_adder, a_adder, mark,
+                        visit_cnt, wave_walk):
+    _ck(lib().f2n_early_stop_votes_ex(_stream(), _i(n_rays), _p(pts_se, "i32"), _p(f0, "f32"), _i(f0_stride), _p(dt, "f32"),
+                                      _p(weights, "f32"), _p(alphas, "f32"), _p(mask, "i32"), _p(kept, "i32"), _i(w_adder.numel()),
+                                      _p(anchors, "i32"), _i(anchor_stride), _p(w_adder, "i32"), _p(a_adder, "i32"), _p(mark, "i32"),
+                                      _p(visit_cnt, "i32"), _i(wave_walk)), "f2n_early_stop_votes_ex")
+
+
 def oct_mark_visit(n_rays, pts_se, anchors, anchor_stride, weights, alphas, w_adder, a_adder, mark, visit_cnt):
     _ck(lib().f2n_oct_mark_visit(_stream(), _i(n_rays), _i(w_adder.numel()), _p(pts_se, "i32"), _p(anchors, "i32"), _i(anchor_stride),
                                  _p(weights, "f32"), _p(alphas, "f32"), _p(w_adder, "i32"), _p(a_adder, "i32"),
@@ -506,7 +516,7 @@
     _ck(lib().f2n_compact_samples_src(_stream(), _i(n_rays), _p(old_se, "i32"), _p(new_se, "i32"), _p(mask, "i32"),
                                       _p(pts, "f32"), _p(dirs, "f32"), _p(dt, "f32"), _p(t, "f32"), _p(anchors, "i32"),
                                       _p(o_pts, "f32"), _p(o_dirs, "f32"), _p(o_dt, "f32"), _p(o_t, "f32"),
-                                      _p(o_anchors, "i32"), _p(o_src, "i32"), _p(o_vol, "i32", True), _p(ray_val, "i32", True),
+                                      _p(o_anchors, "i32", True), _p(o_src, "i32"), _p(o_vol, "i32", True), _p(ray_val, "i32", True),
                                       _p(o_ray_val, "i32", True)), "f2n_compact_samples_src")
 
 
@@ -729,6 +739,15 @@
                                   _i(n_edge), _i(feat_dim), _p(edge_feats, "f32", True), _p(dedge_feats, "f32", True),
                                   _p(colors, "f32"), _p(weights, "f32"), _p(drgb, "f32"), _p(df0, "f32"), _i(df0_stride),
                                   _p(out_losses, "f32"), _i(1 if defer_reduce else 0)), "f2n_composite_train")
+
+
+def composite_train_ex(n_rays, se, f0, f0_stride, dt, t, rgb, bg, gt, var_w, disp_w, tv_w, gs_progress, n_edge, feat_dim, edge_feats,
+                       dedge_feats, colors, weights, drgb, df0, df0_stride, out_losses, wave_walk, defer_reduce=False):
+    _ck(lib().f2n_composite_train_ex(_stream(), _i(n_rays), _p(se, "i32"), _p(f0, "f32"), _i(f0_stride), _p(dt, "f32"), _p(t, "f32"),
+                                     _p(rgb, "f32"), _p(bg, "f32"), _p(gt, "f32"), _f(var_w), _f(disp_w), _f(tv_w), _f(gs_progress),
+                                     _i(n_edge), _i(feat_dim), _p(edge_feats, "f32", True), _p(dedge_feats, "f32", True),
+                                     _p(colors, "f32"), _p(weights, "f32"), _p(drgb, "f32"), _p(df0, "f32"), _i(df0_stride),
+                                     _p(out_losses, "f32"), _i(1 if defer_reduce else 0), _i(wave_walk)), "f2n_composite_train_ex")
 
 
 def nonfinite_flags(n_a, a, n_b, b, flags, mirror=None):
diff --git a/f2-nerf_amd/csrc/host/PersSampler.cpp b/f2-nerf_amd/csrc/host/PersSampler.cpp
--- a/f2-nerf_amd/csrc/host/PersSampler.cpp
+++ b/f2-nerf_amd/csrc/host/PersSampler.cpp
@@ -345,13 +345,13 @@
 }
 
 void PersSampler::EarlyStopAndVote(const SampleResultFlex& sample_result, const float* f0, Tensor& weights, Tensor& alphas, Tensor& mask,
-                                   Tensor& kept) {
+                                   Tensor& kept, int wave_walk) {
   const int n_nodes = pers_octree_->n_nodes_;
   const int n_rays = sample_result.pts_idx_bounds.size(0);
   Tensor& occ = VoteBuffer();
-  F2N_TIMED_CALL("early_stop", f2n_early_stop_votes(CurStream(), n_rays, I32P(sample_result.pts_idx_bounds), f0, 1, F32P(sample_result.dt),
+  F2N_TIMED_CALL("early_stop", f2n_early_stop_votes_ex(CurStream(), n_rays, I32P(sample_result.pts_idx_bounds), f0, 1, F32P(sample_result.dt),
                               F32P(weights), F32P(alphas), I32P(mask), I32P(kept), n_nodes, I32P(sample_result.anchors), 3, I32P(occ),
-                              I32P(occ) + n_nodes, I32P(occ) + 2 * (int64_t) n_nodes, I32P(occ) + 3 * (int64_t) n_nodes));
+                              I32P(occ) + n_nodes, I32P(occ) + 2 * (int64_t) n_nodes, I32P(occ) + 3 * (int64_t) n_nodes, wave_walk));
 }
 
 void PersSampler::FinishOctUpdate(const ScanArgs* scan) {
diff --git a/f2-nerf_amd/csrc/host/PersSampler.h b/f2-nerf_amd/csrc/host/PersSampler.h
--- a/f2-nerf_amd/csrc/host/PersSampler.h
+++ b/f2-nerf_amd/csrc/host/PersSampler.h
@@ -108,7 +108,7 @@
   void UpdateOctNodes(const SampleResultFlex& sample_result, const Tensor& sampled_weights,
                       const Tensor& sampled_alpha) override;
   void EarlyStopAndVote(const SampleResultFlex& sample_result, const float* f0, Tensor& weights, Tensor& alphas, Tensor& mask,
-                        Tensor& kept);
+                        Tensor& kept, int wave_walk = 0);
   struct ScanArgs {
     int n = 0;
     const int32_t* counts = nullptr;
diff --git a/f2-nerf_amd/csrc/host/Renderer.cpp b/f2-nerf_amd/csrc/host/Renderer.cpp
--- a/f2-nerf_amd/csrc/host/Renderer.cpp
+++ b/f2-nerf_amd/csrc/host/Renderer.cpp
@@ -351,7 +351,7 @@
     }
     Tensor weights = torch::empty({n_all_pts}, DevF32()), alphas = torch::empty({n_all_pts}, DevF32());
     Tensor mask = torch::empty({n_all_pts}, DevI32()), kept = torch::empty({n_rays}, DevI32());
-    if (train) ps->EarlyStopAndVote(sample_result_, f0p, weights, alphas, mask, kept);
+    if (train) ps->EarlyStopAndVote(sample_result_, f0p, weights, alphas, mask, kept, ray_walk_wave_);
     else F2N_TIMED_CALL("early_stop", f2n_early_stop(st, n_rays, I32P(sample_result_.pts_idx_bounds), f0p, 1, F32P(sample_result_.dt),
                             F32P(weights), F32P(alphas), I32P(mask), I32P(kept)));
     const bool octree_first = train && async_count;
@@ -434,7 +434,8 @@
     es.dirs = torch::empty({n_kept, 3}, DevF32());
     es.dt = torch::empty({n_kept}, DevF32());
     es.t = torch::empty({n_kept}, DevF32());
-    es.anchors = torch::empty({n_kept, 3}, DevI32());
+    const bool want_anchors = !(train && fr.dyn);
+    if (want_anchors) es.anchors = torch::empty({n_kept, 3}, DevI32());
     es.first_oct_dis = sample_result_.first_oct_dis;
     es.pts_idx_bounds = new_se;
     src_rows = torch::empty({std::max(n_kept, 1)}, DevI32());
@@ -448,7 +449,7 @@
     F2N_TIMED_CALL("compact_samples", f2n_compact_samples_src(st, n_rays, I32P(sample_result_.pts_idx_bounds), I32P(new_se), I32P(mask),
                                  F32P(sample_result_.pts), F32P(sample_result_.dirs), F32P(sample_result_.dt),
                                  F32P(sample_result_.t), I32P(sample_result_.anchors), F32P(pts_all) + 3 * so, F32P(es.dirs),
-                                 F32P(es.dt), F32P(es.t), I32P(es.anchors), I32P(src_rows), I32P(vol_all) + so,
+                                 F32P(es.dt), F32P(es.t), want_anchors ? I32P(es.anchors) : nullptr, I32P(src_rows), I32P(vol_all) + so,
                                  want_emb ? I32P(emb_contig) : nullptr, want_emb ? I32P(fr.sample_emb_idx) : nullptr));
     if (train) {
       if (!fr.dyn) {
diff --git a/f2-nerf_amd/csrc/host/Renderer.h b/f2-nerf_amd/csrc/host/Renderer.h
--- a/f2-nerf_amd/csrc/host/Renderer.h
+++ b/f2-nerf_amd/csrc/host/Renderer.h
@@ -264,6 +264,7 @@
   void DigestTap(int tap, const Tensor& t);
   bool async_count_ = false;
   bool prepass_feat_reuse_ = true;
+  int ray_walk_wave_ = F2N_RAY_WALK_WAVE_DEFAULT;
   bool keep_prepass_outputs_ = false;
   int64_t n_feat_reuse_steps_ = 0;
   bool count_pending_ = false;
diff --git a/f2-nerf_amd/csrc/host/RendererTrain.cpp b/f2-nerf_amd/csrc/host/RendererTrain.cpp
--- a/f2-nerf_amd/csrc/host/RendererTrain.cpp
+++ b/f2-nerf_amd/csrc/host/RendererTrain.cpp
@@ -96,10 +96,10 @@
   Tensor dfeat = torch::empty({n, F2N_MLP_OUT_PAD}, DevF32());
   Tensor drgb = torch::empty({std::max(n_kept, 1), 3}, DevF32());
   if (fr.dyn) {
-    F2N_TIMED_CALL("composite_train", f2n_composite_train(st, n_rays, I32P(es.pts_idx_bounds), F32P(f0c), 1, F32P(es.dt), F32P(es.t), F32P(rgb),
+    F2N_TIMED_CALL("composite_train", f2n_composite_train_ex(st, n_rays, I32P(es.pts_idx_bounds), F32P(f0c), 1, F32P(es.dt), F32P(es.t), F32P(rgb),
                                  F32P(bg), F32P(gt), var_w, disp_w, tv_w, gdp->gradient_scaling_progress_, n_edge, F2N_MLP_OUT_PAD,
                                  n_edge > 0 ? F32P(feat) + F2N_MLP_OUT_PAD * eo : nullptr, n_edge > 0 ? F32P(dfeat) + F2N_MLP_OUT_PAD * eo : nullptr,
-                                 F32P(colors), F32P(weights), F32P(drgb), F32P(df0c), 1, F32P(out.losses), 1));
+                                 F32P(colors), F32P(weights), F32P(drgb), F32P(df0c), 1, F32P(out.losses), 1, ray_walk_wave_));
   } else {
     Tensor disparity = torch::empty({n_rays}, DevF32()), depth = torch::empty({n_rays}, DevF32());
     Tensor var = torch::empty({n_rays}, DevF32());
diff --git a/f2-nerf_amd/csrc/host/bindings.cpp b/f2-nerf_amd/csrc/host/bindings.cpp
--- a/f2-nerf_amd/csrc/host/bindings.cpp
+++ b/f2-nerf_amd/csrc/host/bindings.cpp
@@ -710,6 +710,9 @@
       .def_property("prepass_feat_reuse",
                     [](ExpRunner& r) { return r.renderer_->prepass_feat_reuse_; },
                     [](ExpRunner& r, bool on) { r.renderer_->prepass_feat_reuse_ = on; })
+      .def_property("ray_walk_wave",
+                    [](ExpRunner& r) { return r.renderer_->ray_walk_wave_; },
+                    [](ExpRunner& r, int setting) { r.renderer_->ray_walk_wave_ = setting; })
       .def_property_readonly("prepass_reuse_steps", [](ExpRunner& r) { return r.renderer_->n_feat_reuse_steps_; })
       .def_readwrite("spec_start_without_event", &ExpRunner::spec_start_without_event_)
       .def_readwrite("draws_off_main", &ExpRunner::draws_off_main_)
diff --git a/f2-nerf_amd/csrc/render.hip b/f2-nerf_amd/csrc/render.hip
--- a/f2-nerf_amd/csrc/render.hip
+++ b/f2-nerf_amd/csrc/render.hip
@@ -71,7 +71,10 @@
       for (int c = 0; c < 3; c++) {
         o_pts[3 * (size_t) k + c] = pts[3 * (size_t) i + c];
         o_dirs[3 * (size_t) k + c] = dirs[3 * (size_t) i + c];
-        o_anchors[3 * (size_t) k + c] = anchors[3 * (size_t) i + c];
+      }
+      if (o_anchors != nullptr) {
+#pragma unroll
+        for (int c = 0; c < 3; c++) o_anchors[3 * (size_t) k + c] = anchors[3 * (size_t) i + c];
       }
       o_dt[k] = dt[i];
       o_t[k] = t[i];
@@ -316,6 +319,146 @@
 
 
 #define F2N_CT_TERMS 8
+template <int W, bool COLORS_IN>
+__device__ __forceinline__ void f2n_ct_forward(int s, int e, int c, const float* __restrict__ f0, int f0_stride, const float* __restrict__ dt,
+                                               const float* __restrict__ t, const float* __restrict__ rgb, float* __restrict__ weights,
+                                               float& acc, float (&col)[3], float& disp, float& dep, float& wv_m, float& wv_ws) {
+  acc = 0.f, col[0] = col[1] = col[2] = 0.f, disp = 0.f, dep = 0.f, wv_m = 0.f, wv_ws = 1e-6f;
+  struct In {
+    float f0, dt, t, c0, c1, c2;
+  };
+  auto fetch = [&](int i) {
+    In r;
+    r.f0 = f0[(size_t) i * f0_stride];
+    r.dt = dt[i];
+    r.t = t[i];
+    if (!COLORS_IN) {
+      r.c0 = rgb[3 * (size_t) i];
+      r.c1 = rgb[3 * (size_t) i + 1];
+      r.c2 = rgb[3 * (size_t) i + 2];
+    } else {
+      r.c0 = r.c1 = r.c2 = 0.f;
+    }
+    return r;
+  };
+  In nxt = {0.f, 0.f, 0.f, 0.f, 0.f, 0.f};
+  if (s < e) nxt = fetch(min(s + c, e - 1));
+  for (int base = s; base < e; base += W) {
+    const int i = base + c;
+    const bool in = i < e;
+    const In cur = nxt;
+    if (base + W < e) nxt = fetch(min(i + W, e - 1));
+    float sec = 0.f, tt = 1.f, cr[3] = {0.f, 0.f, 0.f};
+    if (in) {
+      sec = expf(cur.f0 - F2N_DENSITY_SHIFT) * cur.dt;
+      tt = cur.t + F2N_T_BIAS;
+      cr[0] = cur.c0; cr[1] = cur.c1; cr[2] = cur.c2;
+    }
+    const float alpha = 1.f - expf(-sec);
+    float excl;
+    f2n_chain1x<W>(sec, acc, excl);
+    const float trans = expf(-excl);
+    const float w = in ? trans * alpha : 0.f;
+    if (in) weights[i] = w;
+    const float x_disp = w / tt, x_dep = w * tt, x_m = w * ((float) (i - s) / 16.f);
+    if (!COLORS_IN) {
+      f2n_chain4<W>(w * cr[0], w * cr[1], w * cr[2], x_disp, col[0], col[1], col[2], disp);
+      f2n_chain3<W>(x_dep, x_m, w, dep, wv_m, wv_ws);
+    } else {
+      f2n_chain4<W>(x_disp, x_dep, x_m, w, disp, dep, wv_m, wv_ws);
+    }
+  }
+  acc = f2n_group_last<W>(acc);
+#pragma unroll
+  for (int k = 0; k < 3; k++) col[k] = f2n_group_last<W>(col[k]);
+  disp = f2n_group_last<W>(disp);
+  dep = f2n_group_last<W>(dep);
+  wv_m = f2n_group_last<W>(wv_m);
+  wv_ws = f2n_group_last<W>(wv_ws);
+}
+template <int W>
+__device__ __forceinline__ void f2n_ct_weight_var(int s, int e, int c, const float* weights, float wv_mean, float& var, float& wv_tmp) {
+  var = 0.f, wv_tmp = 0.f;
+  float n_w = weights[min(s + c, e - 1)];
+  for (int base = 0; base + s < e; base += W) {
+    const int i = base + c;
+    const float c_w = n_w;
+    if (base + W + s < e) n_w = weights[min(i + W + s, e - 1)];
+    const float b = (float) i / 16.f - wv_mean;
+    const float wi = i + s < e ? c_w : 0.f;
+    f2n_chain2<W>(wi * b * b, wi * 2.f * b, var, wv_tmp);
+  }
+  var = f2n_group_last<W>(var);
+  wv_tmp = f2n_group_last<W>(wv_tmp);
+}
+struct F2nCtRay {
+  float dC[3], dDisp, dDepW, wv_dv, wv_mean, wv_tmp, wv_ws, d_total;
+};
+template <int W>
+__device__ __forceinline__ void f2n_ct_backward(int s, int e, int c, float acc, const F2nCtRay& q, const float* __restrict__ f0, int f0_stride,
+                                                const float* __restrict__ dt, const float* __restrict__ t, const float* __restrict__ rgb,
+                                                float gs_progress, float* __restrict__ drgb, float* __restrict__ df0, int df0_stride) {
+  struct RIn {
+    float f0, dt, t, c0, c1, c2;
+  };
+  auto rfetch = [&](int i) {
+    RIn r;
+    r.f0 = f0[(size_t) i * f0_stride];
+    r.dt = dt[i];
+    r.t = t[i];
+    r.c0 = rgb[3 * (size_t) i];
+    r.c1 = rgb[3 * (size_t) i + 1];
+    r.c2 = rgb[3 * (size_t) i + 2];
+    return r;
+  };
+  float suffix = 0.f;
+  RIn rn = rfetch(max(e - 1 - c, s));
+  for (int hi = e; hi > s; hi -= W) {
+    const int i = hi - 1 - c;
+    const bool in = i >= s;
+    const RIn rc = rn;
+    if (hi - W > s) rn = rfetch(max(i - W, s));
+    float x = 0.f, dti = 0.f, sigma = 0.f, tt = 1.f, c0 = 0.f, c1 = 0.f, c2 = 0.f;
+    if (in) {
+      x = rc.f0 - F2N_DENSITY_SHIFT;
+      sigma = expf(x);
+      dti = rc.dt;
+      tt = rc.t + F2N_T_BIAS;
+      c0 = rc.c0; c1 = rc.c1; c2 = rc.c2;
+    }
+    const float sec = in ? sigma * dti : 0.f;
+    f2n_chain1<W>(-sec, acc);
+    const float acc_i = acc;
+    const float trans = expf(-acc_i);
+    const float ems = expf(-sec);
+    const float alpha = 1.f - ems;
+    const float w = trans * alpha;
+    float dw = (q.dC[0] * c0 + q.dC[1] * c1 + q.dC[2] * c2) + q.dDisp / tt + q.dDepW * tt;
+    if (in) {
+      const float r = (float) (i - s) / 16.f, b = r - q.wv_mean;
+      dw += q.wv_dv * (b * b + q.wv_tmp * -r / q.wv_ws);
+    }
+    const float d_acc = in ? -dw * w : 0.f;
+    float suf_i;
+    f2n_chain1x<W>(d_acc, suffix, suf_i);
+    if (in) {
+      const float d_sec = dw * trans * ems + suf_i + q.d_total;
+      float d_sigma = d_sec * dti;
+      float g0 = q.dC[0] * w, g1 = q.dC[1] * w, g2 = q.dC[2] * w;
+      if (gs_progress < 1.f) {
+        const float a = ((float) (i - s) + .5f) / (float) (e - s);
+        const float sc = gs_progress + (1.f - gs_progress) * a * a;
+        d_sigma *= sc;
+        g0 *= sc; g1 *= sc; g2 *= sc;
+      }
+      drgb[3 * (size_t) i] = g0;
+      drgb[3 * (size_t) i + 1] = g1;
+      drgb[3 * (size_t) i + 2] = g2;
+      df0[(size_t) i * df0_stride] = d_sigma * expf(fminf(fmaxf(x, -100.f), 5.f));
+    }
+  }
+}
+
 template <bool COLORS_IN>
 __global__ __launch_bounds__(256) void composite_train_kernel(
     int n_rays, const int32_t* __restrict__ se, const float* __restrict__ f0, int f0_stride, const float* __restrict__ dt,
@@ -323,7 +466,7 @@
     float var_w, float disp_w, float tv_w, float gs_progress, int n_edge, int feat_dim, const float* __restrict__ edge,
     float* __restrict__ dedge, float* __restrict__ colors, float* __restrict__ weights, float* __restrict__ drgb,
     float* __restrict__ df0, int df0_stride, float* __restrict__ partials, float* __restrict__ out_losses, int ray_blocks,
-    const float* __restrict__ colors_in) {
+    const float* __restrict__ colors_in, int wave_walk) {
   F2N_RAISE_PRIO();
   __shared__ float s_terms[F2N_ROW_RAYS_PER_BLOCK][4];
   __shared__ float s_tv[256];
@@ -364,59 +507,25 @@
     s = se[2 * ray];
     e = se[2 * ray + 1];
   }
-  float acc = 0.f, col[3] = {0.f, 0.f, 0.f}, disp = 0.f, dep = 0.f, wv_m = 0.f, wv_ws = 1e-6f;
-  {
-    struct In {
-      float f0, dt, t, c0, c1, c2;
-    };
-    auto fetch = [&](int i) {
-      In r;
-      r.f0 = f0[(size_t) i * f0_stride];
-      r.dt = dt[i];
-      r.t = t[i];
-      if (!COLORS_IN) {
-        r.c0 = rgb[3 * (size_t) i];
-        r.c1 = rgb[3 * (size_t) i + 1];
-        r.c2 = rgb[3 * (size_t) i + 2];
-      } else {
-        r.c0 = r.c1 = r.c2 = 0.f;
-      }
-      return r;
-    };
-    In nxt = {0.f, 0.f, 0.f, 0.f, 0.f, 0.f};
-    if (s < e) nxt = fetch(min(s + c, e - 1));
-    for (int base = s; base < e; base += 16) {
-      const int i = base + c;
-      const bool in = i < e;
-      const In cur = nxt;
-      if (base + 16 < e) nxt = fetch(min(i + 16, e - 1));
-      float sec = 0.f, tt = 1.f, cr[3] = {0.f, 0.f, 0.f};
-      if (in) {
-        sec = expf(cur.f0 - F2N_DENSITY_SHIFT) * cur.dt;
-        tt = cur.t + F2N_T_BIAS;
-        cr[0] = cur.c0; cr[1] = cur.c1; cr[2] = cur.c2;
-      }
-      const float alpha = 1.f - expf(-sec);
-      float excl;
-      f2n_row_chain1x(sec, acc, excl);
-      const float trans = expf(-excl);
-      const float w = in ? trans * alpha : 0.f;
-      if (in) weights[i] = w;
-      const float x_disp = w / tt, x_dep = w * tt, x_m = w * ((float) (i - s) / 16.f);
-      if (!COLORS_IN) {
-        f2n_row_chain4(w * cr[0], w * cr[1], w * cr[2], x_disp, col[0], col[1], col[2], disp);
-        f2n_row_chain3(x_dep, x_m, w, dep, wv_m, wv_ws);
-      } else {
-        f2n_row_chain4(x_disp, x_dep, x_m, w, disp, dep, wv_m, wv_ws);
-      }
-    }
-    acc = f2n_row_last(acc);
-#pragma unroll
-    for (int k = 0; k < 3; k++) col[k] = f2n_row_last(col[k]);
-    disp = f2n_row_last(disp);
-    dep = f2n_row_last(dep);
-    wv_m = f2n_row_last(wv_m);
-    wv_ws = f2n_row_last(wv_ws);
+  const int lane = threadIdx.x & 63, wrow = lane >> 4;
+  const unsigned wide = COLORS_IN ? 0u : f2n_wave_pick(e - s, wave_walk);
+  const int re = ((wide >> wrow) & 1u) ? s : e;
+  float acc, col[3], disp, dep, wv_m, wv_ws;
+  f2n_ct_forward<16, COLORS_IN>(s, re, c, f0, f0_stride, dt, t, rgb, weights, acc, col, disp, dep, wv_m, wv_ws);
+  float var = 0.f, wv_tmp = 0.f;
+  if (!COLORS_IN && wide != 0u) {
+    for (int r = 0; r < 4; r++) {
+      if (!((wide >> r) & 1u)) continue;
+      const int ws = __shfl(s, 16 * r, 64), we = __shfl(e, 16 * r, 64);
+      float a_acc, a_col[3], a_disp, a_dep, a_m, a_ws, a_var = 0.f, a_tmp = 0.f;
+      f2n_ct_forward<64, false>(ws, we, lane, f0, f0_stride, dt, t, rgb, weights, a_acc, a_col, a_disp, a_dep, a_m, a_ws);
+      if (ws < we) f2n_ct_weight_var<64>(ws, we, lane, weights, a_m / a_ws, a_var, a_tmp);
+      if (wrow == r) {
+        acc = a_acc, disp = a_disp, dep = a_dep, wv_m = a_m, wv_ws = a_ws, var = a_var, wv_tmp = a_tmp;
+#pragma unroll
+        for (int k = 0; k < 3; k++) col[k] = a_col[k];
+      }
+    }
   }
   if (COLORS_IN && live) {
 #pragma unroll
@@ -436,34 +545,22 @@
 #pragma unroll
   for (int k = 0; k < 3; k++) pred[k] = col[k] + last_trans * bgc[k];
   if (live && c < 3) colors[3 * ray + c] = c == 0 ? pred[0] : c == 1 ? pred[1] : pred[2];
-  float var = 0.f, wv_tmp = 0.f;
   const float wv_mean = wv_m / wv_ws;
-  if (s < e) {
-    float n_w = weights[min(s + c, e - 1)];
-    for (int base = 0; base + s < e; base += 16) {
-      const int i = base + c;
-      const float c_w = n_w;
-      if (base + 16 + s < e) n_w = weights[min(i + 16 + s, e - 1)];
-      const float b = (float) i / 16.f - wv_mean;
-      const float wi = i + s < e ? c_w : 0.f;
-      f2n_row_chain2(wi * b * b, wi * 2.f * b, var, wv_tmp);
-    }
-    var = f2n_row_last(var);
-    wv_tmp = f2n_row_last(wv_tmp);
-  }
+  if (s < re) f2n_ct_weight_var<16>(s, re, c, weights, wv_mean, var, wv_tmp);
   const float inv_col = 1.f / (float) max(3 * n_rays, 1), inv_ray = 1.f / (float) max(n_rays, 1);
-  float dC[3], t_col = 0.f, t_mse = 0.f;
+  F2nCtRay q;
+  float t_col = 0.f, t_mse = 0.f;
 #pragma unroll
   for (int k = 0; k < 3; k++) {
     const float d = pred[k] - gtc[k];
     const float r = sqrtf(d * d + 1e-4f);
     t_col += r;
     t_mse += d * d;
-    dC[k] = d / r * inv_col;
+    q.dC[k] = d / r * inv_col;
   }
   const float r_var = sqrtf(var + 1e-2f);
-  const float wv_dv = var_w * .5f / r_var * inv_ray;
-  const float dDisp = disp_w * 2.f * disp * inv_ray;
+  q.wv_dv = var_w * .5f / r_var * inv_ray;
+  q.dDisp = disp_w * 2.f * disp * inv_ray;
   if (c == 0) {
     s_terms[row][0] = live ? t_col * inv_col : 0.f;
     s_terms[row][1] = live ? r_var * inv_ray : 0.f;
@@ -483,70 +580,33 @@
     partials[(size_t) blockIdx.x * F2N_CT_TERMS + k] =
         k == 0 ? sc + sv * var_w + sd * disp_w : k == 1 ? sc : k == 2 ? sv : k == 3 ? sd : k == 5 ? sm : 0.f;
   }
-  if (s >= e) return;
   const float dep_sum = dep;
   const float denom = 1.f - last_trans + 1e-4f;
   const float dDep = 0.f;
-  const float d_last = (dC[0] * bgc[0] + dC[1] * bgc[1] + dC[2] * bgc[2]) + dDep * dep_sum / (denom * denom);
-  const float d_total = -last_trans * d_last;
-  const float dDepW = dDep / denom;
-  struct RIn {
-    float f0, dt, t, c0, c1, c2;
-  };
-  auto rfetch = [&](int i) {
-    RIn r;
-    r.f0 = f0[(size_t) i * f0_stride];
-    r.dt = dt[i];
-    r.t = t[i];
-    r.c0 = rgb[3 * (size_t) i];
-    r.c1 = rgb[3 * (size_t) i + 1];
-    r.c2 = rgb[3 * (size_t) i + 2];
-    return r;
-  };
-  float suffix = 0.f;
-  RIn rn = rfetch(max(e - 1 - c, s));
-  for (int hi = e; hi > s; hi -= 16) {
-    const int i = hi - 1 - c;
-    const bool in = i >= s;
-    const RIn rc = rn;
-    if (hi - 16 > s) rn = rfetch(max(i - 16, s));
-    float x = 0.f, dti = 0.f, sigma = 0.f, tt = 1.f, c0 = 0.f, c1 = 0.f, c2 = 0.f;
-    if (in) {
-      x = rc.f0 - F2N_DENSITY_SHIFT;
-      sigma = expf(x);
-      dti = rc.dt;
-      tt = rc.t + F2N_T_BIAS;
-      c0 = rc.c0; c1 = rc.c1; c2 = rc.c2;
-    }
-    const float sec = in ? sigma * dti : 0.f;
-    f2n_row_chain1(-sec, acc);
-    const float acc_i = acc;
-    const float trans = expf(-acc_i);
-    const float ems = expf(-sec);
-    const float alpha = 1.f - ems;
-    const float w = trans * alpha;
-    float dw = (dC[0] * c0 + dC[1] * c1 + dC[2] * c2) + dDisp / tt + dDepW * tt;
-    if (in) {
-      const float r = (float) (i - s) / 16.f, b = r - wv_mean;
-      dw += wv_dv * (b * b + wv_tmp * -r / wv_ws);
-    }
-    const float d_acc = in ? -dw * w : 0.f;
-    float suf_i;
-    f2n_row_chain1x(d_acc, suffix, suf_i);
-    if (in) {
-      const float d_sec = dw * trans * ems + suf_i + d_total;
-      float d_sigma = d_sec * dti;
-      float g0 = dC[0] * w, g1 = dC[1] * w, g2 = dC[2] * w;
-      if (gs_progress < 1.f) {
-        const float a = ((float) (i - s) + .5f) / (float) (e - s);
-        const float sc = gs_progress + (1.f - gs_progress) * a * a;
-        d_sigma *= sc;
-        g0 *= sc; g1 *= sc; g2 *= sc;
-      }
-      drgb[3 * (size_t) i] = g0;
-      drgb[3 * (size_t) i + 1] = g1;
-      drgb[3 * (size_t) i + 2] = g2;
-      df0[(size_t) i * df0_stride] = d_sigma * expf(fminf(fmaxf(x, -100.f), 5.f));
+  const float d_last = (q.dC[0] * bgc[0] + q.dC[1] * bgc[1] + q.dC[2] * bgc[2]) + dDep * dep_sum / (denom * denom);
+  q.d_total = -last_trans * d_last;
+  q.dDepW = dDep / denom;
+  q.wv_mean = wv_mean;
+  q.wv_tmp = wv_tmp;
+  q.wv_ws = wv_ws;
+  if (s < re) f2n_ct_backward<16>(s, re, c, acc, q, f0, f0_stride, dt, t, rgb, gs_progress, drgb, df0, df0_stride);
+  if (!COLORS_IN && wide != 0u) {
+    for (int r = 0; r < 4; r++) {
+      if (!((wide >> r) & 1u)) continue;
+      const int src = 16 * r;
+      const int ws = __shfl(s, src, 64), we = __shfl(e, src, 64);
+      if (ws >= we) continue;
+      F2nCtRay a;
+#pragma unroll
+      for (int k = 0; k < 3; k++) a.dC[k] = __shfl(q.dC[k], src, 64);
+      a.dDisp = __shfl(q.dDisp, src, 64);
+      a.dDepW = __shfl(q.dDepW, src, 64);
+      a.wv_dv = __shfl(q.wv_dv, src, 64);
+      a.wv_mean = __shfl(q.wv_mean, src, 64);
+      a.wv_tmp = __shfl(q.wv_tmp, src, 64);
+      a.wv_ws = __shfl(q.wv_ws, src, 64);
+      a.d_total = __shfl(q.d_total, src, 64);
+      f2n_ct_backward<64>(ws, we, lane, __shfl(acc, src, 64), a, f0, f0_stride, dt, t, rgb, gs_progress, drgb, df0, df0_stride);
     }
   }
 }
@@ -808,7 +868,7 @@
                         const float* t, const float* rgb, const float* bg, const float* gt_colors, float var_w, float disp_w, float tv_w,
                         float grad_scaling_progress, int n_edge, int feat_dim, const float* edge_feats, float* dedge_feats,
                         float* colors, float* weights, float* drgb, float* df0, int df0_stride, float* out_losses, int defer_reduce,
-                        const float* colors_in) {
+                        const float* colors_in, int wave_walk) {
   if (n_rays < 1 || f0_stride < 1 || df0_stride < 1 || n_edge < 0 || (n_edge > 0 && (edge_feats == nullptr || feat_dim < 1)) ||
       out_losses == nullptr)
     return F2N_ERR_INVALID_ARG;
@@ -822,25 +882,35 @@
   if (colors_in != nullptr)
     hipLaunchKernelGGL(composite_train_kernel<true>, dim3(blocks), dim3(256), 0, (hipStream_t) stream, n_rays, pts_start_end, f0, f0_stride, dt,
                        t, rgb, bg, gt_colors, var_w, disp_w, tv_w, grad_scaling_progress, n_edge, feat_dim, edge_feats, dedge_feats, colors,
-                       weights, drgb, df0, df0_stride, partials, out_losses, ray_blocks, colors_in);
+                       weights, drgb, df0, df0_stride, partials, out_losses, ray_blocks, colors_in, wave_walk);
   else
 #endif
   hipLaunchKernelGGL(composite_train_kernel<false>, dim3(blocks), dim3(256), 0, (hipStream_t) stream, n_rays, pts_start_end, f0, f0_stride, dt,
                      t, rgb, bg, gt_colors, var_w, disp_w, tv_w, grad_scaling_progress, n_edge, feat_dim, edge_feats, dedge_feats, colors,
-                     weights, drgb, df0, df0_stride, partials, out_losses, ray_blocks, colors_in);
+                     weights, drgb, df0, df0_stride, partials, out_losses, ray_blocks, colors_in, wave_walk);
   const int rc = f2n_launch_status();
   if (rc != F2N_OK) return rc;
   if (defer_reduce) return f2n_defer_reduction(F2N_CT_TERMS, blocks, partials, out_losses);
   return f2n_reduce_partials(stream, F2N_CT_TERMS, blocks, partials, out_losses);
 }
 
+int f2n_composite_train_ex(void* stream, int n_rays, const int32_t* pts_start_end, const float* f0, int f0_stride, const float* dt,
+                           const float* t, const float* rgb, const float* bg, const float* gt_colors, float var_w, float disp_w, float tv_w,
+                           float grad_scaling_progress, int n_edge, int feat_dim, const float* edge_feats, float* dedge_feats,
+                           float* colors, float* weights, float* drgb, float* df0, int df0_stride, float* out_losses, int defer_reduce,
+                           int wave_walk) {
+  return f2n_composite_train_impl(stream, n_rays, pts_start_end, f0, f0_stride, dt, t, rgb, bg, gt_colors, var_w, disp_w, tv_w,
+                                  grad_scaling_progress, n_edge, feat_dim, edge_feats, dedge_feats, colors, weights, drgb, df0, df0_stride,
+                                  out_losses, defer_reduce, nullptr, wave_walk);
+}
+
 int f2n_composite_train(void* stream, int n_rays, const int32_t* pts_start_end, const float* f0, int f0_stride, const float* dt,
                         const float* t, const float* rgb, const float* bg, const float* gt_colors, float var_w, float disp_w, float tv_w,
                         float grad_scaling_progress, int n_edge, int feat_dim, const float* edge_feats, float* dedge_feats,
                         float* colors, float* weights, float* drgb, float* df0, int df0_stride, float* out_losses, int defer_reduce) {
-  return f2n_composite_train_impl(stream, n_rays, pts_start_end, f0, f0_stride, dt, t, rgb, bg, gt_colors, var_w, disp_w, tv_w,
-                                  grad_scaling_progress, n_edge, feat_dim, edge_feats, dedge_feats, colors, weights, drgb, df0, df0_stride,
-                                  out_losses, defer_reduce, nullptr);
+  return f2n_composite_train_ex(stream, n_rays, pts_start_end, f0, f0_stride, dt, t, rgb, bg, gt_colors, var_w, disp_w, tv_w,
+                                grad_scaling_progress, n_edge, feat_dim, edge_feats, dedge_feats, colors, weights, drgb, df0, df0_stride,
+                                out_losses, defer_reduce, 0);
 }
 
 #if F2N_DEBUG_BUILD
@@ -849,7 +919,7 @@
                                         float var_w, float disp_w, float tv_w, float grad_scaling_progress, float* colors, float* weights,
                                         float* drgb, float* df0, float* out_losses, const float* colors_in) {
   return f2n_composite_train_impl(stream, n_rays, pts_start_end, f0, f0_stride, dt, t, rgb, bg, gt_colors, var_w, disp_w, tv_w,
-                                  grad_scaling_progress, 0, 16, nullptr, nullptr, colors, weights, drgb, df0, 1, out_losses, 0, colors_in);
+                                  grad_scaling_progress, 0, 16, nullptr, nullptr, colors, weights, drgb, df0, 1, out_losses, 0, colors_in, 0);
 }
 #endif
 
diff --git a/f2-nerf_amd/csrc/rows_dev.h b/f2-nerf_amd/csrc/rows_dev.h
--- a/f2-nerf_amd/csrc/rows_dev.h
+++ b/f2-nerf_amd/csrc/rows_dev.h
@@ -83,8 +83,131 @@
   f2n_row_chain1(x3, p3);
 }
 #endif
+#if defined(__HIP_DEVICE_COMPILE__)
+#define F2N_WDPP_STEP_(P, X) "v_add_f32_dpp " P ", " P ", " X " wave_shr:1 row_mask:0xf bank_mask:0xf\n\t"
+#define F2N_WDPP_HEAD_(P, X) "v_add_f32_dpp " P ", " P ", " X " wave_ror:1 row_mask:0xf bank_mask:0xf\n\t"
+#define F2N_REP63_(S) F2N_REP15_(S) F2N_REP15_(S) F2N_REP15_(S) F2N_REP15_(S) S S S
+__device__ __forceinline__ void f2n_wave_chain1(float x, float& p) {
+  asm volatile("s_nop 4\n\t" F2N_WDPP_HEAD_("%0", "%1") "s_nop 1\n\t" F2N_REP63_(F2N_WDPP_STEP_("%0", "%1") "s_nop 1\n\t") : "+v"(p) : "v"(x));
+}
+__device__ __forceinline__ void f2n_wave_chain1x(float x, float& p, float& excl) {
+  asm volatile("s_nop 4\n\t"
+               "v_mov_b32_dpp %1, %0 wave_ror:1 row_mask:0xf bank_mask:0xf\n\t" F2N_WDPP_HEAD_("%0", "%2") "s_nop 1\n\t" F2N_REP63_(
+                   F2N_WDPP_STEP_("%0", "%2") "s_nop 1\n\t") "v_mov_b32_dpp %1, %0 wave_shr:1 row_mask:0xf bank_mask:0xf\n\t"
+                                                             "s_nop 1\n\t"
+               : "+v"(p), "=&v"(excl)
+               : "v"(x));
+}
+__device__ __forceinline__ void f2n_wave_chain2(float x0, float x1, float& p0, float& p1) {
+  asm volatile("s_nop 4\n\t" F2N_WDPP_HEAD_("%0", "%2") F2N_WDPP_HEAD_("%1", "%3") "s_nop 0\n\t" F2N_REP63_(
+                   F2N_WDPP_STEP_("%0", "%2") F2N_WDPP_STEP_("%1", "%3") "s_nop 0\n\t") "s_nop 0\n\t"
+               : "+v"(p0), "+v"(p1)
+               : "v"(x0), "v"(x1));
+}
+__device__ __forceinline__ void f2n_wave_chain3(float x0, float x1, float x2, float& p0, float& p1, float& p2) {
+  asm volatile("s_nop 4\n\t" F2N_WDPP_HEAD_("%0", "%3") F2N_WDPP_HEAD_("%1", "%4") F2N_WDPP_HEAD_("%2", "%5") F2N_REP63_(
+                   F2N_WDPP_STEP_("%0", "%3") F2N_WDPP_STEP_("%1", "%4") F2N_WDPP_STEP_("%2", "%5")) "s_nop 1\n\t"
+               : "+v"(p0), "+v"(p1), "+v"(p2)
+               : "v"(x0), "v"(x1), "v"(x2));
+}
+__device__ __forceinline__ void f2n_wave_chain4(float x0, float x1, float x2, float x3, float& p0, float& p1, float& p2, float& p3) {
+  asm volatile("s_nop 4\n\t" F2N_WDPP_HEAD_("%0", "%4") F2N_WDPP_HEAD_("%1", "%5") F2N_WDPP_HEAD_("%2", "%6") F2N_WDPP_HEAD_("%3", "%7") F2N_REP63_(
+                   F2N_WDPP_STEP_("%0", "%4") F2N_WDPP_STEP_("%1", "%5") F2N_WDPP_STEP_("%2", "%6") F2N_WDPP_STEP_("%3", "%7")) "s_nop 1\n\t"
+               : "+v"(p0), "+v"(p1), "+v"(p2), "+v"(p3)
+               : "v"(x0), "v"(x1), "v"(x2), "v"(x3));
+}
+#else
+__device__ __forceinline__ float f2n_wave_shr1(float v) {
+  return __int_as_float(__builtin_amdgcn_update_dpp(0, __float_as_int(v), 0x138, 0xF, 0xF, false));
+}
+__device__ __forceinline__ float f2n_wave_seq_scan(float x, float carry, int l) {
+  float p = carry + x;
+  for (int k = 1; k < 64; k++) {
+    const float t = f2n_wave_shr1(p) + x;
+    p = (l == 0) ? p : t;
+  }
+  return p;
+}
+__device__ __forceinline__ void f2n_wave_chain1(float x, float& p) { p = f2n_wave_seq_scan(x, __shfl(p, 63, 64), (int) (threadIdx.x & 63)); }
+__device__ __forceinline__ void f2n_wave_chain1x(float x, float& p, float& excl) {
+  const int l = threadIdx.x & 63;
+  const float carry = __shfl(p, 63, 64);
+  p = f2n_wave_seq_scan(x, carry, l);
+  const float prev = f2n_wave_shr1(p);
+  excl = l == 0 ? carry : prev;
+}
+__device__ __forceinline__ void f2n_wave_chain2(float x0, float x1, float& p0, float& p1) {
+  f2n_wave_chain1(x0, p0);
+  f2n_wave_chain1(x1, p1);
+}
+__device__ __forceinline__ void f2n_wave_chain3(float x0, float x1, float x2, float& p0, float& p1, float& p2) {
+  f2n_wave_chain1(x0, p0);
+  f2n_wave_chain1(x1, p1);
+  f2n_wave_chain1(x2, p2);
+}
+__device__ __forceinline__ void f2n_wave_chain4(float x0, float x1, float x2, float x3, float& p0, float& p1, float& p2, float& p3) {
+  f2n_wave_chain1(x0, p0);
+  f2n_wave_chain1(x1, p1);
+  f2n_wave_chain1(x2, p2);
+  f2n_wave_chain1(x3, p3);
+}
+#endif
 __device__ __forceinline__ float f2n_row_last(float v) { return __shfl(v, 15, 16); }
 __device__ __forceinline__ float f2n_row_exclusive(float incl, float carry, int c) {
   const float prev = f2n_row_shr1(incl);
   return c == 0 ? carry : prev;
 }
+
+template <int W> __device__ __forceinline__ void f2n_chain1(float x, float& p) {
+  if constexpr (W == 64) f2n_wave_chain1(x, p); else f2n_row_chain1(x, p);
+}
+template <int W> __device__ __forceinline__ void f2n_chain1x(float x, float& p, float& excl) {
+  if constexpr (W == 64) f2n_wave_chain1x(x, p, excl); else f2n_row_chain1x(x, p, excl);
+}
+template <int W> __device__ __forceinline__ void f2n_chain2(float x0, float x1, float& p0, float& p1) {
+  if constexpr (W == 64) f2n_wave_chain2(x0, x1, p0, p1); else f2n_row_chain2(x0, x1, p0, p1);
+}
+template <int W> __device__ __forceinline__ void f2n_chain3(float x0, float x1, float x2, float& p0, float& p1, float& p2) {
+  if constexpr (W == 64) f2n_wave_chain3(x0, x1, x2, p0, p1, p2); else f2n_row_chain3(x0, x1, x2, p0, p1, p2);
+}
+template <int W> __device__ __forceinline__ void f2n_chain4(float x0, float x1, float x2, float x3, float& p0, float& p1, float& p2, float& p3) {
+  if constexpr (W == 64) f2n_wave_chain4(x0, x1, x2, x3, p0, p1, p2, p3); else f2n_row_chain4(x0, x1, x2, x3, p0, p1, p2, p3);
+}
+template <int W> __device__ __forceinline__ float f2n_group_last(float v) { return __shfl(v, W - 1, W); }
+
+__device__ __forceinline__ unsigned f2n_wave_pick(int len, int setting) {
+  if (setting == 0) return 0u;
+  int L[4];
+#pragma unroll
+  for (int r = 0; r < 4; r++) L[r] = __shfl(len, 16 * r, 64);
+  unsigned mask = 0u;
+  if (setting < 0) {
+#pragma unroll
+    for (int r = 0; r < 4; r++) mask |= L[r] > 16 ? 1u << r : 0u;
+  } else {
+    int rank[4], S[5] = {0, 0, 0, 0, 0};
+#pragma unroll
+    for (int r = 0; r < 4; r++) {
+      rank[r] = 0;
+#pragma unroll
+      for (int j = 0; j < 4; j++) rank[r] += (L[j] > L[r] || (L[j] == L[r] && j < r)) ? 1 : 0;
+    }
+#pragma unroll
+    for (int r = 0; r < 4; r++)
+#pragma unroll
+      for (int k = 0; k < 4; k++) S[k] = rank[r] == k ? L[r] : S[k];
+    int best = 0, best_cost = 8 * ((S[0] + 15) >> 4), wave_cost = 0;
+#pragma unroll
+    for (int k = 1; k <= 4; k++) {
+      wave_cost += ((S[k - 1] + 63) >> 6) * setting;
+      const int cost = wave_cost + 8 * ((S[k] + 15) >> 4);
+      if (cost < best_cost) {
+        best_cost = cost;
+        best = k;
+      }
+    }
+#pragma unroll
+    for (int r = 0; r < 4; r++) mask |= rank[r] < best ? 1u << r : 0u;
+  }
+  return (unsigned) __builtin_amdgcn_readfirstlane((int) mask);
+}
diff --git a/f2-nerf_amd/csrc/sampler.hip b/f2-nerf_amd/csrc/sampler.hip
--- a/f2-nerf_amd/csrc/sampler.hip
+++ b/f2-nerf_amd/csrc/sampler.hip
@@ -786,8 +786,9 @@
   if (cc < visits) atomicMax(cnt + node, visits);
   if (cm != 1) mark[node] = 1;
 }
+template <int W = 16>
 __device__ __forceinline__ void f2n_votes_flush_row(const uint2* list, int n, int c, int32_t* w_adder, int32_t* a_adder, int32_t* mark, int32_t* cnt) {
-  for (int k = c; k < n; k += 16) {
+  for (int k = c; k < n; k += W) {
     const uint2 r = list[k];
     f2n_vote_global(w_adder, a_adder, mark, cnt, (int) r.x, (r.y & 1u) ? 512 : -1, (r.y & 2u) ? 32 : -1, (int) (r.y >> 2));
   }
@@ -800,6 +801,7 @@
   if (mark != nullptr) mark[node] = 1;
 }
 
+template <int W = 16>
 __device__ __forceinline__ void f2n_ray_votes(int s, int e, int c, float mw, float ma, const int32_t* __restrict__ anchors,
                                               int anchor_stride, const float* weights, const float* alphas, int32_t* w_adder,
                                               int32_t* a_adder, int32_t* mark, int32_t* cnt, uint2* vote_list = nullptr) {
@@ -808,7 +810,7 @@
   const float a_thres = fminf((float) ((double) ma * 0.1), (float) 0.02);
   float carry_w = 0.f, carry_a = 0.f;
   int carry_start = s, carry_node = -1;
-  auto rot1 = [](int v) { return __builtin_amdgcn_update_dpp(0, v, 0x121, 0xF, 0xF, false); };
+  auto rot1 = [](int v) { return __builtin_amdgcn_update_dpp(0, v, W == 64 ? 0x13C : 0x121, 0xF, 0xF, false); };
   struct Chunk {
     int node;
     float w, a;
@@ -821,8 +823,9 @@
     q.a = alphas[j];
     return q;
   };
-  Chunk q0 = fetch_chunk(s), q1 = fetch_chunk(s + 16), q2 = fetch_chunk(s + 32), q3 = fetch_chunk(s + 48);
-  for (int base = s; base < e; base += 16) {
+  Chunk q0 = fetch_chunk(s), q1 = fetch_chunk(s + W), q2 = fetch_chunk(s + 2 * W), q3 = fetch_chunk(s + 3 * W);
+  const int cr = c & 15;
+  for (int base = s; base < e; base += W) {
     const int i = base + c;
     const bool in = i < e;
     const int ic = in ? i : e - 1;
@@ -831,11 +834,11 @@
     q0 = q1;
     q1 = q2;
     q2 = q3;
-    q3 = fetch_chunk(base + 64);
+    q3 = fetch_chunk(base + 4 * W);
     const int n_node = q0.node;
-    const int prev = __builtin_amdgcn_update_dpp(base > s ? carry_node : -1, node, 0x111, 0xF, 0xF, false);
-    const int nx0 = __builtin_amdgcn_update_dpp(0, n_node, 0x12F, 0xF, 0xF, false);
-    const int nxt = __builtin_amdgcn_update_dpp(nx0, node, 0x101, 0xF, 0xF, false);
+    const int prev = __builtin_amdgcn_update_dpp(base > s ? carry_node : -1, node, W == 64 ? 0x138 : 0x111, 0xF, 0xF, false);
+    const int nx0 = __builtin_amdgcn_update_dpp(0, n_node, W == 64 ? 0x134 : 0x12F, 0xF, 0xF, false);
+    const int nxt = __builtin_amdgcn_update_dpp(nx0, node, W == 64 ? 0x130 : 0x101, 0xF, 0xF, false);
     const int next = ic + 1 < e ? nxt : -1;
     const bool head = node != prev;
     float cw = fmaxf(0.f, c_w), ca = fmaxf(0.f, c_a);
@@ -852,30 +855,42 @@
     const float ta = __int_as_float(__builtin_amdgcn_update_dpp(0, __float_as_int(ca), 0x110 + K, 0xF, 0xF, false)); \
     const int ts = __builtin_amdgcn_update_dpp((int) 0x80000000, start, 0x110 + K, 0xF, 0xF, false);              \
     const int tf = __builtin_amdgcn_update_dpp(1, f, 0x110 + K, 0xF, 0xF, false);                                 \
-    if (c >= K && f == 0) {                                                                    \
+    if (cr >= K && f == 0) {                                                                   \
       cw = fmaxf(cw, tw);                                                                      \
       ca = fmaxf(ca, ta);                                                                      \
       start = max(start, ts);                                                                  \
     }                                                                                          \
-    if (c >= K) f |= tf;                                                                       \
+    if (cr >= K) f |= tf;                                                                      \
   }
     F2N_SEGMAX_STEP(1)
     F2N_SEGMAX_STEP(2)
     F2N_SEGMAX_STEP(4)
     F2N_SEGMAX_STEP(8)
 #undef F2N_SEGMAX_STEP
+    if constexpr (W == 64) {
+#pragma unroll
+      for (int r = 1; r < 4; r++) {
+        const float tw = __shfl(cw, 16 * r - 1, 64), ta = __shfl(ca, 16 * r - 1, 64);
+        const int ts = __shfl(start, 16 * r - 1, 64);
+        if ((c >> 4) == r && f == 0) {
+          cw = fmaxf(cw, tw);
+          ca = fmaxf(ca, ta);
+          start = max(start, ts);
+        }
+      }
+    }
     const bool votes = in && node != next;
     if (vote_list == nullptr) {
       if (votes) f2n_vote(w_adder, a_adder, mark, cnt, node, cw, ca, w_thres, a_thres, ic - start + 1);
     } else {
-      const unsigned row_bits = (unsigned) ((__ballot(votes) >> (threadIdx.x & 48)) & 0xFFFFull);
-      const int n_new = __popc(row_bits);
+      const unsigned long long row_bits = W == 64 ? __ballot(votes) : ((__ballot(votes) >> (threadIdx.x & 48)) & 0xFFFFull);
+      const int n_new = __popcll(row_bits);
       if (n_queued + n_new > F2N_VOTE_CAP) {
-        f2n_votes_flush_row(vote_list, n_queued, c, w_adder, a_adder, mark, cnt);
+        f2n_votes_flush_row<W>(vote_list, n_queued, c, w_adder, a_adder, mark, cnt);
         n_queued = 0;
       }
       if (votes)
-        vote_list[n_queued + __popc(row_bits & ((1u << c) - 1u))] =
+        vote_list[n_queued + __popcll(row_bits & ((1ull << c) - 1ull))] =
             make_uint2((unsigned) node, (cw > w_thres ? 1u : 0u) | (ca > a_thres ? 2u : 0u) | ((unsigned) (ic - start + 1) << 2));
       n_queued += n_new;
     }
@@ -884,7 +899,7 @@
     carry_start = rot1(start);
     carry_node = rot1(node);
   }
-  if (vote_list != nullptr) f2n_votes_flush_row(vote_list, n_queued, c, w_adder, a_adder, mark, cnt);
+  if (vote_list != nullptr) f2n_votes_flush_row<W>(vote_list, n_queued, c, w_adder, a_adder, mark, cnt);
 }
 
 __device__ __forceinline__ void f2n_votes_lds_init(int32_t* s_votes, int n_nodes) {
@@ -945,12 +960,60 @@
   if (USE_LDS) f2n_votes_lds_flush(s_votes, n_nodes, g_w_adder, g_a_adder, g_mark, g_cnt);
 }
 
+template <int W>
+__device__ __forceinline__ void f2n_early_stop_walk(int s, int e, int c, const float* __restrict__ f0, int f0_stride,
+                                                    const float* __restrict__ dt, float* weights, float* alphas,
+                                                    int32_t* __restrict__ mask, int& cnt, float& mw, float& ma) {
+  float acc = 0.f;
+  cnt = 0;
+  mw = 0.f;
+  ma = 0.f;
+  float n_f0 = 0.f, n_dt = 0.f;
+  if (s < e) {
+    const int i = min(s + c, e - 1);
+    n_f0 = f0[(size_t) i * f0_stride];
+    n_dt = dt[i];
+  }
+  for (int base = s; base < e; base += W) {
+    const int i = base + c;
+    const bool in = i < e;
+    const float c_f0 = n_f0, c_dt = n_dt;
+    if (base + W < e) {
+      const int j = min(i + W, e - 1);
+      n_f0 = f0[(size_t) j * f0_stride];
+      n_dt = dt[j];
+    }
+    float sec = 0.f;
+    if (in) sec = expf(c_f0 - F2N_DENSITY_SHIFT) * c_dt;
+    const float alpha = 1.f - expf(-sec);
+    float excl;
+    f2n_chain1x<W>(sec, acc, excl);
+    const float trans = expf(-excl);
+    const int m = (in && trans > F2N_T_EPS) ? 1 : 0;
+    if (in) {
+      const float w = trans * alpha;
+      weights[i] = w;
+      alphas[i] = alpha;
+      mask[i] = m;
+      mw = fmaxf(mw, w);
+      ma = fmaxf(ma, alpha);
+    }
+    cnt += m;
+  }
+#pragma unroll
+  for (int off = W / 2; off >= 1; off >>= 1) {
+    cnt += __shfl_xor(cnt, off, W);
+    mw = fmaxf(mw, __shfl_xor(mw, off, W));
+    ma = fmaxf(ma, __shfl_xor(ma, off, W));
+  }
+}
+
 template <bool USE_LDS>
 __global__ void early_stop_votes_kernel(int n_rays, int n_nodes, const int32_t* __restrict__ se, const float* __restrict__ f0,
                                         int f0_stride, const float* __restrict__ dt, float* weights, float* alphas,
                                         int32_t* __restrict__ mask, int32_t* __restrict__ kept,
                                         const int32_t* __restrict__ anchors, int anchor_stride, int32_t* g_w_adder,
-                                        int32_t* g_a_adder, int32_t* g_mark, int32_t* g_cnt) {
+                                        int32_t* g_a_adder, int32_t* g_mark, int32_t* g_cnt, int wave_walk) {
   extern __shared__ int32_t s_votes[];
   __shared__ uint2 s_vote_list[USE_LDS ? 1 : 16 * F2N_VOTE_CAP];
   int32_t* w_adder = USE_LDS ? s_votes : g_w_adder;
@@ -965,50 +1028,29 @@
     s = se[2 * ray];
     e = se[2 * ray + 1];
   }
-  float acc = 0.f, mw = 0.f, ma = 0.f;
-  int cnt = 0;
-  float n_f0 = 0.f, n_dt = 0.f;
-  if (s < e) {
-    const int i = min(s + c, e - 1);
-    n_f0 = f0[(size_t) i * f0_stride];
-    n_dt = dt[i];
-  }
-  for (int base = s; base < e; base += 16) {
-    const int i = base + c;
-    const bool in = i < e;
-    const float c_f0 = n_f0, c_dt = n_dt;
-    if (base + 16 < e) {
-      const int j = min(i + 16, e - 1);
-      n_f0 = f0[(size_t) j * f0_stride];
-      n_dt = dt[j];
-    }
-    float sec = 0.f;
-    if (in) sec = expf(c_f0 - F2N_DENSITY_SHIFT) * c_dt;
-    const float alpha = 1.f - expf(-sec);
-    float excl;
-    f2n_row_chain1x(sec, acc, excl);
-    const float trans = expf(-excl);
-    const int m = (in && trans > F2N_T_EPS) ? 1 : 0;
-    if (in) {
-      const float w = trans * alpha;
-      weights[i] = w;
-      alphas[i] = alpha;
-      mask[i] = m;
-      mw = fmaxf(mw, w);
-      ma = fmaxf(ma, alpha);
-    }
-    cnt += m;
-  }
-#pragma unroll
-  for (int off = 8; off >= 1; off >>= 1) {
-    cnt += __shfl_xor(cnt, off, 16);
-    mw = fmaxf(mw, __shfl_xor(mw, off, 16));
-    ma = fmaxf(ma, __shfl_xor(ma, off, 16));
+  const int lane = threadIdx.x & 63, wrow = lane >> 4;
+  const unsigned wide = f2n_wave_pick(e - s, wave_walk);
+  const int re = ((wide >> wrow) & 1u) ? s : e;
+  float mw, ma;
+  int cnt;
+  f2n_early_stop_walk<16>(s, re, c, f0, f0_stride, dt, weights, alphas, mask, cnt, mw, ma);
+  if (s < re)
+    f2n_ray_votes<16>(s, re, c, mw, ma, anchors, anchor_stride, weights, alphas, w_adder, a_adder, mark, cnt_v,
+                      USE_LDS ? nullptr : s_vote_list + (threadIdx.x >> 4) * F2N_VOTE_CAP);
+  if (wide != 0u) {
+    for (int r = 0; r < 4; r++) {
+      if (!((wide >> r) & 1u)) continue;
+      const int ws = __shfl(s, 16 * r, 64), we = __shfl(e, 16 * r, 64);
+      float w_mw, w_ma;
+      int w_cnt;
+      f2n_early_stop_walk<64>(ws, we, lane, f0, f0_stride, dt, weights, alphas, mask, w_cnt, w_mw, w_ma);
+      if (ws < we)
+        f2n_ray_votes<64>(ws, we, lane, w_mw, w_ma, anchors, anchor_stride, weights, alphas, w_adder, a_adder, mark, cnt_v,
+                          USE_LDS ? nullptr : s_vote_list + ((threadIdx.x >> 6) * 4 + r) * F2N_VOTE_CAP);
+      if (wrow == r) cnt = w_cnt;
+    }
   }
   if (ray < n_rays && c == 0) kept[ray] = cnt;
-  if (s < e)
-    f2n_ray_votes(s, e, c, mw, ma, anchors, anchor_stride, weights, alphas, w_adder, a_adder, mark, cnt_v,
-                  USE_LDS ? nullptr : s_vote_list + (threadIdx.x >> 4) * F2N_VOTE_CAP);
   if (USE_LDS) f2n_votes_lds_flush(s_votes, n_nodes, g_w_adder, g_a_adder, g_mark, g_cnt);
 }
 
@@ -1519,22 +1561,29 @@
   return f2n_launch_status();
 }
 
-int f2n_early_stop_votes(void* stream, int n_rays, const int32_t* pts_start_end, const float* f0, int f0_stride, const float* dt,
+int f2n_early_stop_votes_ex(void* stream, int n_rays, const int32_t* pts_start_end, const float* f0, int f0_stride, const float* dt,
                          float* weights, float* alphas, int32_t* mask, int32_t* kept, int n_nodes, const int32_t* anchors,
-                         int anchor_stride, int32_t* w_adder, int32_t* a_adder, int32_t* mark, int32_t* visit_cnt) {
+                         int anchor_stride, int32_t* w_adder, int32_t* a_adder, int32_t* mark, int32_t* visit_cnt, int wave_walk) {
   if (n_rays < 0 || n_nodes < 1 || anchor_stride < 2 || f0_stride < 1) return F2N_ERR_INVALID_ARG;
   if (n_rays == 0) return F2N_OK;
   const size_t lds = sizeof(int32_t) * 3 * (size_t) n_nodes;
   if (lds <= 60 * 1024) {
     hipLaunchKernelGGL(early_stop_votes_kernel<true>, dim3(f2n_div_up(n_rays, 64)), dim3(1024), lds, (hipStream_t) stream, n_rays,
                        n_nodes, pts_start_end, f0, f0_stride, dt, weights, alphas, mask, kept, anchors, anchor_stride, w_adder,
-                       a_adder, mark, visit_cnt);
+                       a_adder, mark, visit_cnt, wave_walk);
   } else {
     hipLaunchKernelGGL(early_stop_votes_kernel<false>, dim3(f2n_div_up(n_rays, 16)), dim3(256), 0, (hipStream_t) stream, n_rays,
                        n_nodes, pts_start_end, f0, f0_stride, dt, weights, alphas, mask, kept, anchors, anchor_stride, w_adder,
-                       a_adder, mark, visit_cnt);
-  }
-  return f2n_launch_status();
+                       a_adder, mark, visit_cnt, wave_walk);
+  }
+  return f2n_launch_status();
+}
+
+int f2n_early_stop_votes(void* stream, int n_rays, const int32_t* pts_start_end, const float* f0, int f0_stride, const float* dt,
+                         float* weights, float* alphas, int32_t* mask, int32_t* kept, int n_nodes, const int32_t* anchors,
+                         int anchor_stride, int32_t* w_adder, int32_t* a_adder, int32_t* mark, int32_t* visit_cnt) {
+  return f2n_early_stop_votes_ex(stream, n_rays, pts_start_end, f0, f0_stride, dt, weights, alphas, mask, kept, n_nodes, anchors,
+                                 anchor_stride, w_adder, a_adder, mark, visit_cnt, 0);
 }
 
 int f2n_oct_update_stats(void* stream, int n_nodes, int32_t* w_adder, int32_t* a_adder, int32_t* mark, int32_t* w_stats,
diff --git a/include/f2n_abi.h b/include/f2n_abi.h
--- a/include/f2n_abi.h
+++ b/include/f2n_abi.h
@@ -263,6 +263,11 @@
 int f2n_early_stop_votes(void* stream, int n_rays, const int32_t* pts_start_end, const float* f0, int f0_stride, const float* dt,
                          float* weights, float* alphas, int32_t* mask, int32_t* kept, int n_nodes, const int32_t* anchors,
                          int anchor_stride, int32_t* w_adder, int32_t* a_adder, int32_t* mark, int32_t* visit_cnt);
+#define F2N_RAY_WALK_WAVE_DEFAULT 0
+#define F2N_RAY_WALK_WAVE_FITTED 16
+int f2n_early_stop_votes_ex(void* stream, int n_rays, const int32_t* pts_start_end, const float* f0, int f0_stride, const float* dt,
+                            float* weights, float* alphas, int32_t* mask, int32_t* kept, int n_nodes, const int32_t* anchors,
+                            int anchor_stride, int32_t* w_adder, int32_t* a_adder, int32_t* mark, int32_t* visit_cnt, int wave_walk);
 
 int f2n_compact_samples(void* stream, int n_rays, const int32_t* old_start_end, const int32_t* new_start_end,
                         const int32_t* mask, const float* pts, const float* dirs, const float* dt, const float* t,
@@ -271,7 +276,7 @@
 int f2n_compact_samples_src(void* stream, int n_rays, const int32_t* old_start_end, const int32_t* new_start_end,
                             const int32_t* mask, const float* pts, const float* dirs, const float* dt, const float* t,
                             const int32_t* anchors, float* o_pts, float* o_dirs, float* o_dt, float* o_t,
-                            int32_t* o_anchors, int32_t* o_src ,
+                            int32_t* o_anchors , int32_t* o_src ,
                             int32_t* o_vol ,
                             const int32_t* ray_val ,
                             int32_t* o_ray_val );
@@ -401,6 +406,11 @@
                         float grad_scaling_progress, int n_edge, int feat_dim, const float* edge_feats ,
                         float* dedge_feats , float* colors, float* weights, float* drgb, float* df0, int df0_stride,
                         float* out_losses , int defer_reduce);
+int f2n_composite_train_ex(void* stream, int n_rays, const int32_t* pts_start_end, const float* f0, int f0_stride, const float* dt,
+                           const float* t, const float* rgb, const float* bg, const float* gt_colors, float var_w, float disp_w, float tv_w,
+                           float grad_scaling_progress, int n_edge, int feat_dim, const float* edge_feats ,
+                           float* dedge_feats , float* colors, float* weights, float* drgb, float* df0, int df0_stride,
+                           float* out_losses , int defer_reduce, int wave_walk);
 
 int f2n_nonfinite_flags(void* stream, int n_a, const float* a, int n_b, const float* b, int32_t* flags );
 int f2n_nonfinite_flags_ex(void* stream, int n_a, const float* a, int n_b, const float* b, int32_t* flags ,
```

New measurement: 644.7 million ray-samples/s. 0.966x the previous value.
